# magic-research/vector_quantization

Hardware: AMD Instinct MI355X
Metric: quantized tokens/sec, VQGAN quantizer forward K=16384 D=256 (higher is better)
Workload: dtype f16+f32; 1 GPU; VQGAN K=16384 D=256, 256x256 images -> 16x16 tokens, bf16 latents, VQGANQuantizer.forward of the drop-in nn.Module, eval mode (prepare+argmin+gather+STE+loss); images_per_gpu=2048, parallelism=dp1 (independent shards, no data-path collective)

## Files before the change

### include/vqhip.h

```cpp
#ifndef VQHIP_H_
#define VQHIP_H_

#include <stddef.h>
#include <stdint.h>

#ifdef __cplusplus
extern "C" {
#endif

#define VQHIP_VERSION 600

#define VQHIP_METRIC_L2 0
#define VQHIP_METRIC_COS 1
#define VQHIP_METRIC_COS_BF16 5

#define VQHIP_DTYPE_F32 0
#define VQHIP_DTYPE_BF16 1

#define VQHIP_OK 0
#define VQHIP_EINVAL (-22)
#define VQHIP_ELAUNCH (-5)
#define VQHIP_ERCCL (-71)

int vqhip_version(void);
// ... 104 lines not shown
                          int64_t N, int64_t K, int D, int metric, int64_t *col_idx, void *ws, int64_t ws_bytes, void *stream);
int vqhip_cvq_pack(const int32_t *hist, int64_t numel, const void *x, int x_dtype, const int64_t *col_idx, const int32_t *count,
                   int64_t cap, int64_t K, int D, float *packed, void *stream);
int vqhip_cvq_apply(const float *w_in, float *w_out, const float *p_in, float *p_out, const int32_t *hist, int64_t numel,
                    const void *x, int x_dtype, const int64_t *col_idx, const float *packed, int world, const int32_t *slot,
                    int64_t cap, int64_t K, int D, float ema_decay, float eps, void *stream);
#define VQHIP_SYNC_MAX_ROWS (1 << 24)
int vqhip_cvq_col_keys(const void *x, int x_dtype, const float *e, const int32_t *rows, const int32_t *count, int64_t cap,
                       const int64_t *col_idx, int64_t N, int64_t K, int D, int metric, int rank, int64_t *keys, void *stream);
int vqhip_cvq_pack_sync(const int32_t *hist, int64_t numel, const void *x, int x_dtype, const int64_t *keys, const int32_t *count,
                        int64_t cap, int rank, int64_t K, int D, float *packed, void *stream);
int vqhip_allreduce_min_i64(int64_t *buf, int64_t n, void *comm, void *stream);
#define VQHIP_STEP_BEFORE_EXCHANGE 1
#define VQHIP_STEP_AFTER_EXCHANGE 2
#define VQHIP_STEP_ALL 3
#define VQHIP_STEP_PACK_SYNC 4
typedef struct vqhip_cvq_forward_t {
    int64_t struct_bytes;
    int64_t N, K;
    int32_t D, x_dtype, metric, world;
    float ema_decay, eps, beta;
    int32_t phases, exchange, list_ready, prefetch;
    int32_t anchor_sync, rank;
    int64_t cap;
    const void *x;
    const float *w_in, *p_in;
    float *w_out, *p_out;
    int32_t *rows, *slot, *count;
    int32_t *count_host;
    void *count_event;
    void *comm;
    void *cb; int64_t cb_bytes;
    int64_t *idx; int32_t *hist; float *xq;
    float *packed; int64_t packed_floats;
    float *z_ste, *mse; void *scratch16;
    void *ws; int64_t ws_bytes;
    int64_t cap_used, exchange_floats;
    unsigned long long *early_word_host;
    int32_t *early_seq_dev;
    int64_t *keys;
} vqhip_cvq_forward_t;
int64_t vqhip_cvq_forward_ws_bytes(int64_t N, int64_t K, int D, int64_t cap_max);
int vqhip_cvq_forward(vqhip_cvq_forward_t *args, void *stream);

typedef struct vqhip_vqkd_forward_t {
    int64_t struct_bytes;
    int64_t N, K;
    int32_t D, x_dtype, metric, world;
    float ema_decay;
    int32_t phases, exchange, ordered, tail, reserved0;
    const void *x;
    const float *w_in;
    float *w_mid, *w_out;
    float *xn, *xq;
    void *comm;
    void *cb; int64_t cb_bytes;
    int64_t *idx; int32_t *hist;
    float *packed; int64_t packed_floats;
    float *z_ste, *mse; void *scratch16;
    void *ws; int64_t ws_bytes;
    int64_t exchange_floats;
} vqhip_vqkd_forward_t;
int64_t vqhip_vqkd_forward_ws_bytes(int64_t N, int64_t K, int D);
int vqhip_vqkd_forward(vqhip_vqkd_forward_t *args, void *stream);
int vqhip_vqkd_backward(const void *x, int x_dtype, const float *xn, const float *w, const int64_t *idx, int64_t N, int D,
                        const float *g_zste, const float *g_loss, float *grad_x, void *stream);

typedef struct vqhip_vq_forward_t {
    int64_t struct_bytes;
    int64_t N, K;
    int32_t D, x_dtype, metric, normalize;
    float beta;
    int32_t reserved0;
    const void *x;
    const float *w_in;
    float *w_out, *xn;
    void *cb; int64_t cb_bytes;
    int64_t *idx; int32_t *hist; float *xq;
    float *z_ste, *mse; void *scratch16;
    void *ws; int64_t ws_bytes;
} vqhip_vq_forward_t;
int vqhip_vq_forward(vqhip_vq_forward_t *args, void *stream);

int vqhip_gather_rows(const void *x, int x_dtype, const int64_t *row_idx, int64_t K, int D, float *out,
                      void *stream);

int vqhip_diff(const void *a, int a_dtype, const void *b, int b_dtype, int64_t n, float scale,
               const float *scale_dev , float *out, double *sse,
               void *stream);
int vqhip_vq_backward(const void *x, int x_dtype, const float *e, const int64_t *idx, int64_t N, int D,
                      const float *g_zste, const float *g_cb, const float *g_cm, float *grad_x, float *grad_w,
                      void *stream);
int vqhip_vq_backward_ex(const void *x, int x_dtype, const float *e, const int64_t *idx, int64_t N, int D,
                         const float *g_zste, const float *g_cb, const float *g_cm, const float *g_comb, float beta,
                         float *grad_x, float *grad_w, void *stream);
int vqhip_vq_backward_map(const void *x_rows, int x_dtype, const float *e, const int64_t *idx, int64_t B, int64_t HW, int D,
                          const float *g_map, const float *g_cm, const float *g_comb, float beta, void *grad_map, int grad_dtype,
                          void *stream);
int vqhip_ste(const void *x, int x_dtype, const float *z, int64_t n, float *out, void *stream);
int vqhip_normalize_rows_bwd(const void *v, int dtype, const float *g, int64_t R, int D, float eps, float *gv,
                             void *stream);

int64_t vqhip_order_workspace_bytes(int64_t N, int64_t K);
int64_t vqhip_segsum_workspace_bytes(int64_t N, int D);
int vqhip_token_order(const int64_t *idx, int64_t N, int64_t K, int32_t *counts, int32_t *offsets, int32_t *order, void *ws,
                      int64_t ws_bytes, void *stream);
int vqhip_segsum_rows(const float *src, const int64_t *idx, const int32_t *order, const int32_t *offsets, int64_t N, int64_t K,
                      int D, float *dst, void *ws, int64_t ws_bytes, void *stream);
int vqhip_vq_backward_w_ordered(const void *x, int x_dtype, const float *e, const int64_t *idx, const int32_t *order,
                                const int32_t *offsets, int64_t N, int64_t K, int D, const float *g_cb, float *grad_w, void *ws,
                                int64_t ws_bytes, void *stream);

int vqhip_transpose(const void *in, void *out, int elem_bytes, int64_t B, int R, int C, void *stream);
int vqhip_codebook_metrics(const int64_t *counts, int64_t K, double *out, void *stream);

int vqhip_argmin_stats(const void *ws, int32_t *out, void *stream);

int vqhip_debug_proposal_scores(const void *x, int x_dtype, const void *cb, int64_t N, int64_t K, int D, int metric,
                                float *scores, float *margin, float *scale, void *ws, int64_t ws_bytes, void *stream);

int vqhip_profile_enable(int on);
int vqhip_set_tuning(int key, int value);
int vqhip_profile_collect(double *ms_sum, int64_t *launches);

#ifdef __cplusplus
}
#endif
#endif
```

### vector_quantization_amd/_lib.py

```python
from __future__ import annotations

import ctypes
import os
import subprocess

_HERE = os.path.dirname(os.path.abspath(__file__))
LIB_PATH = os.environ.get('VQHIP_LIB') or os.path.join(_HERE, 'libvqhip.so')

ABI_VERSION = 600
METRIC_L2, METRIC_COS, METRIC_COS_BF16 = 0, 1, 5
DTYPE_F32, DTYPE_BF16 = 0, 1
DTYPE_I32, DTYPE_I64 = 2, 3
LAYOUT_ROWS, LAYOUT_MAP = 0, 1
FSQ_MAX_C = 16

_vp, _i64, _i32, _f32 = ctypes.c_void_p, ctypes.c_int64, ctypes.c_int, ctypes.c_float


class CvqForwardArgs(ctypes.Structure):
    _fields_ = [('struct_bytes', _i64), ('N', _i64), ('K', _i64),
                ('D', _i32), ('x_dtype', _i32), ('metric', _i32), ('world', _i32),
                ('ema_decay', _f32), ('eps', _f32), ('beta', _f32),
                ('phases', _i32), ('exchange', _i32), ('list_ready', _i32), ('prefetch', _i32), ('anchor_sync', _i32), ('rank', _i32),
                ('cap', _i64),
                ('x', _vp), ('w_in', _vp), ('p_in', _vp), ('w_out', _vp), ('p_out', _vp),
                ('rows', _vp), ('slot', _vp), ('count', _vp), ('count_host', _vp), ('count_event', _vp), ('comm', _vp),
                ('cb', _vp), ('cb_bytes', _i64), ('idx', _vp), ('hist', _vp), ('xq', _vp),
                ('packed', _vp), ('packed_floats', _i64),
                ('z_ste', _vp), ('mse', _vp), ('scratch16', _vp),
                ('ws', _vp), ('ws_bytes', _i64),
                ('cap_used', _i64), ('exchange_floats', _i64),
                ('early_word_host', _vp), ('early_seq_dev', _vp), ('keys', _vp)]


class VqkdForwardArgs(ctypes.Structure):
    _fields_ = [('struct_bytes', _i64), ('N', _i64), ('K', _i64),
                ('D', _i32), ('x_dtype', _i32), ('metric', _i32), ('world', _i32),
                ('ema_decay', _f32),
                ('phases', _i32), ('exchange', _i32), ('ordered', _i32), ('tail', _i32), ('reserved0', _i32),
                ('x', _vp), ('w_in', _vp), ('w_mid', _vp), ('w_out', _vp), ('xn', _vp), ('xq', _vp), ('comm', _vp),
                ('cb', _vp), ('cb_bytes', _i64), ('idx', _vp), ('hist', _vp),
                ('packed', _vp), ('packed_floats', _i64),
                ('z_ste', _vp), ('mse', _vp), ('scratch16', _vp),
                ('ws', _vp), ('ws_bytes', _i64),
                ('exchange_floats', _i64)]


class VqForwardArgs(ctypes.Structure):
    _fields_ = [('struct_bytes', _i64), ('N', _i64), ('K', _i64),
                ('D', _i32), ('x_dtype', _i32), ('metric', _i32), ('normalize', _i32),
                ('beta', _f32), ('reserved0', _i32),
                ('x', _vp), ('w_in', _vp), ('w_out', _vp), ('xn', _vp),
                ('cb', _vp), ('cb_bytes', _i64), ('idx', _vp), ('hist', _vp), ('xq', _vp),
                ('z_ste', _vp), ('mse', _vp), ('scratch16', _vp),
                ('ws', _vp), ('ws_bytes', _i64)]


class FsqConstants(ctypes.Structure):
    _fields_ = [('struct_bytes', _i64), ('C', _i32), ('levels', _i32 * FSQ_MAX_C),
                ('shift', _f32 * FSQ_MAX_C), ('scale', _f32 * FSQ_MAX_C)]


STEP_BEFORE_EXCHANGE, STEP_AFTER_EXCHANGE, STEP_ALL, STEP_PACK_SYNC = 1, 2, 3, 4

SIGNATURES = {
    'vqhip_version': (_i32, []),
    'vqhip_last_error': (ctypes.c_char_p, []),
    'vqhip_codebook_bytes': (_i64, [_i64, _i32]),
    'vqhip_codebook_exact_offset': (_i64, [_i64, _i32]),
    'vqhip_encode': (_i32, [_vp, _i32, _vp, _i64, _i64, _i32, _i32, _vp, _i64, _vp, _vp, _vp, _vp, _i64, _vp]),
    'vqhip_encode_ex': (_i32, [_vp, _i32, _vp, _i64, _i64, _i32, _i32, _vp, _i64, _vp, _vp, _vp, _vp, _i64, _i32, _vp]),
    'vqhip_encode_map': (_i32, [_vp, _i32, _vp, _i64, _i64, _i64, _i32, _i32, _vp, _i64, _vp, _vp, _vp, _vp, _vp, _i64, _i32, _vp]),
    'vqhip_gather_ste_map': (_i32, [_vp, _i32, _vp, _vp, _i64, _i64, _i32, _vp, _vp, _f32, _vp, _vp]),
    'vqhip_workspace_bytes': (_i64, [_i64, _i64, _i32]),
    'vqhip_col_workspace_bytes': (_i64, [_i64, _i64, _i32]),
    'vqhip_codebook_prepare': (_i32, [_vp, _i64, _i32, _i32, _vp, _i64, _vp]),
    'vqhip_argmin': (_i32, [_vp, _i32, _vp, _vp, _i64, _i64, _i64, _i32, _i32, _vp, _vp, _vp, _i64, _vp]),
    'vqhip_argmin_exact': (_i32, [_vp, _i32, _vp, _i64, _i64, _i32, _i32, _vp, _vp, _vp, _vp, _i64, _vp]),
    'vqhip_distance': (_i32, [_vp, _i32, _vp, _i64, _i64, _i32, _i32, _vp, _vp, _i64, _vp]),
    'vqhip_col_argmin': (_i32, [_vp, _i32, _vp, _i64, _i64, _i32, _i32, _vp, _vp, _i64, _vp]),
    'vqhip_row_sqnorm': (_i32, [_vp, _i32, _i64, _i32, _vp, _vp]),
    'vqhip_normalize_rows': (_i32, [_vp, _i32, _i64, _i32, _f32, _vp, _vp]),
    'vqhip_gather_ste_loss': (_i32, [_vp, _i32, _vp, _vp, _i64, _i32, _vp, _vp, _vp, _vp]),
    'vqhip_gather_ste_mse': (_i32, [_vp, _i32, _vp, _vp, _i64, _i32, _vp, _vp, _vp, _f32, _vp, _vp]),
    'vqhip_hist': (_i32, [_vp, _i64, _i64, _vp, _vp]),
    'vqhip_hist_i32': (_i32, [_vp, _i64, _i64, _vp, _vp]),
    'vqhip_fsq_encode': (_i32, [ctypes.POINTER(FsqConstants), _vp, _i32, _i32, _i64, _i64, _vp, _vp, _i32, _vp, _vp, _vp]),
    'vqhip_fsq_backward': (_i32, [ctypes.POINTER(FsqConstants), _vp, _i32, _i32, _i64, _i64, _vp, _vp, _vp]),
    'vqhip_fsq_decode': (_i32, [ctypes.POINTER(FsqConstants), _vp, _i32, _i32, _i64, _i64, _vp, _vp]),
    'vqhip_entropy_workspace_bytes': (_i64, [_i64, _i64]),
    'vqhip_entropy_rows': (_i32, [_vp, _i64, _i64, _f32, _vp, _vp, _vp, _i32, _vp, _i64, _vp]),
    'vqhip_entropy_finish': (_i32, [_vp, _vp, _vp, _i64, _i64, _vp, _vp, _vp, _vp]),
    'vqhip_entropy_grad': (_i32, [_vp, _i64, _i64, _f32, _vp, _vp, _vp, _f32, _vp, _i32, _vp, _vp, _i32, _vp, _i64, _vp]),
    'vqhip_scatter_add_rows': (_i32, [_vp, _vp, _i64, _i64, _i32, _vp, _vp]),
    'vqhip_vqkd_update': (_i32, [_vp, _vp, _vp, _i64, _i32, _f32, _i32, _vp]),
    'vqhip_cvq_update': (_i32, [_vp, _vp, _vp, _i64, _vp, _vp, _i64, _i32, _f32, _f32, _i32, _vp]),
    'vqhip_gather_rows': (_i32, [_vp, _i32, _vp, _i64, _i32, _vp, _vp]),
    'vqhip_diff': (_i32, [_vp, _i32, _vp, _i32, _i64, _f32, _vp, _vp, _vp, _vp]),
    'vqhip_vq_backward': (_i32, [_vp, _i32, _vp, _vp, _i64, _i32, _vp, _vp, _vp, _vp, _vp, _vp]),
    'vqhip_vq_backward_ex': (_i32, [_vp, _i32, _vp, _vp, _i64, _i32, _vp, _vp, _vp, _vp, _f32, _vp, _vp, _vp]),
    'vqhip_vq_backward_map': (_i32, [_vp, _i32, _vp, _vp, _i64, _i64, _i32, _vp, _vp, _vp, _f32, _vp, _i32, _vp]),
    'vqhip_ste': (_i32, [_vp, _i32, _vp, _i64, _vp, _vp]),
    'vqhip_normalize_rows_bwd': (_i32, [_vp, _i32, _vp, _i64, _i32, _f32, _vp, _vp]),
    'vqhip_transpose': (_i32, [_vp, _vp, _i32, _i64, _i32, _i32, _vp]),
    'vqhip_codebook_metrics': (_i32, [_vp, _i64, _vp, _vp]),
    'vqhip_argmin_stats': (_i32, [_vp, _vp, _vp]),
    'vqhip_cvq_step': (_i32, [_vp, _vp, _vp, _vp, _vp, _i64, _vp, _i32, _vp, _i64, _i32, _f32, _f32, _vp]),
    'vqhip_cvq_decay': (_i32, [_vp, _i64, _f32, _f32, _vp, _vp]),
    'vqhip_cvq_update_rows': (_i32, [_vp, _vp, _vp, _vp, _i64, _i64, _i32, _f32, _f32, _vp]),
    'vqhip_pack_floats': (_i64, [_i64, _i64, _i32]),
    'vqhip_pack_counts': (_i32, [_vp, _i32, _i64, _i64, _vp, _vp]),
    'vqhip_unpack_counts': (_i32, [_vp, _i64, _vp, _vp]),
    'vqhip_cvq_rows': (_i32, [_vp, _i64, _f32, _f32, _vp, _vp, _vp, _vp]),
    'vqhip_col_rows_workspace_bytes': (_i64, [_i64, _i64, _i32]),
    'vqhip_col_argmin_rows': (_i32, [_vp, _i32, _vp, _vp, _vp, _i64, _i64, _i64, _i32, _i32, _vp, _vp, _i64, _vp]),
    'vqhip_cvq_pack': (_i32, [_vp, _i64, _vp, _i32, _vp, _vp, _i64, _i64, _i32, _vp, _vp]),
    'vqhip_cvq_forward_ws_bytes': (_i64, [_i64, _i64, _i32, _i64]),
    'vqhip_cvq_forward': (_i32, [ctypes.POINTER(CvqForwardArgs), _vp]),
    'vqhip_vqkd_forward_ws_bytes': (_i64, [_i64, _i64, _i32]),
    'vqhip_vqkd_forward': (_i32, [ctypes.POINTER(VqkdForwardArgs), _vp]),
    'vqhip_vq_forward': (_i32, [ctypes.POINTER(VqForwardArgs), _vp]),
    'vqhip_vqkd_backward': (_i32, [_vp, _i32, _vp, _vp, _vp, _i64, _i32, _vp, _vp, _vp, _vp]),
    'vqhip_cvq_apply': (_i32, [_vp, _vp, _vp, _vp, _vp, _i64, _vp, _i32, _vp, _vp, _i32, _vp, _i64, _i64, _i32, _f32, _f32, _vp]),
    'vqhip_cvq_col_keys': (_i32, [_vp, _i32, _vp, _vp, _vp, _i64, _vp, _i64, _i64, _i32, _i32, _i32, _vp, _vp]),
    'vqhip_cvq_pack_sync': (_i32, [_vp, _i64, _vp, _i32, _vp, _vp, _i64, _i32, _i64, _i32, _vp, _vp]),
    'vqhip_allreduce_min_i64': (_i32, [_vp, _i64, _vp, _vp]),
    'vqhip_order_workspace_bytes': (_i64, [_i64, _i64]),
    'vqhip_token_order': (_i32, [_vp, _i64, _i64, _vp, _vp, _vp, _vp, _i64, _vp]),
    'vqhip_segsum_workspace_bytes': (_i64, [_i64, _i32]),
    'vqhip_segsum_rows': (_i32, [_vp, _vp, _vp, _vp, _i64, _i64, _i32, _vp, _vp, _i64, _vp]),
    'vqhip_vq_backward_w_ordered': (_i32, [_vp, _i32, _vp, _vp, _vp, _vp, _i64, _i64, _i32, _vp, _vp, _vp, _i64, _vp]),
    'vqhip_debug_proposal_scores': (_i32, [_vp, _i32, _vp, _i64, _i64, _i32, _i32, _vp, _vp, _vp, _vp, _i64, _vp]),
    'vqhip_rccl_load': (_i32, [ctypes.c_char_p]),
    'vqhip_rccl_unique_id': (_i32, [_vp]),
    'vqhip_rccl_comm_init': (_i32, [ctypes.POINTER(_vp), _i32, _vp, _i32]),
    'vqhip_rccl_comm_destroy': (_i32, [_vp]),
    'vqhip_allreduce_packed': (_i32, [_vp, _i64, _vp, _vp]),
    'vqhip_profile_enable': (_i32, [_i32]),
    'vqhip_set_tuning': (_i32, [_i32, _i32]),
    'vqhip_profile_collect': (_i32, [ctypes.POINTER(ctypes.c_double), ctypes.POINTER(ctypes.c_int64)]),
}

_lib = None


class VqhipError(RuntimeError):
    pass


def build(verbose: bool = False) -> str:
    script = os.path.join(_HERE, 'csrc', 'build.sh')
    res = subprocess.run(['bash', script], capture_output=True, text=True)
    if res.returncode != 0:
        raise VqhipError(f'hipcc build of libvqhip.so failed:\n{res.stdout}\n{res.stderr}')
    if verbose:
        print(res.stdout.strip())
    return LIB_PATH


def lib() -> ctypes.CDLL:
    global _lib
    if _lib is None:
        if not os.path.exists(LIB_PATH):
            raise VqhipError(
                f'{LIB_PATH} not found: build it with vector_quantization_amd/csrc/build.sh '
                '(or __graft_entry__.build()); there is no fallback path')
        L = ctypes.CDLL(LIB_PATH)
# ... 20 lines not shown
```

### vector_quantization_amd/csrc/vqhip.hip

```cpp
#include "vqhip.h"

#include <hip/hip_runtime.h>
#include <stdio.h>
#include <string.h>

#include "vqhip_kernels.h"
#include "vqhip_fsq_kernels.h"
#include "vqhip_entropy_kernels.h"

static thread_local char g_err[256] = "";

static int fail(int code, const char *what, const char *detail = "") {
    snprintf(g_err, sizeof(g_err), "%s%s%s", what, detail[0] ? ": " : "", detail);
    return code;
}

#define VQ_CHECK_LAUNCH(name)                                            \
    do {                                                                 \
        hipError_t err__ = hipGetLastError();                            \
        if (err__ != hipSuccess) return fail(VQHIP_ELAUNCH, name, hipGetErrorString(err__)); \
    } while (0)

#define VQ_HIP(call)                                                     \
    do {                                                                 \
        hipError_t err__ = (call);                                       \
        if (err__ != hipSuccess) return fail(VQHIP_ELAUNCH, #call, hipGetErrorString(err__)); \
    } while (0)

#include <atomic>
#include <mutex>
#include <vector>
static std::atomic<bool> g_prof_on{false};
static std::mutex g_prof_mu;
static std::vector<std::pair<hipEvent_t, hipEvent_t>> g_prof_events;
static size_t g_prof_used = 0;

static long prof_begin(hipStream_t s) {
    if (!g_prof_on.load(std::memory_order_relaxed)) return -1;
    std::lock_guard<std::mutex> lock(g_prof_mu);
    if (g_prof_used == g_prof_events.size()) {
        hipEvent_t a, b;
        if (hipEventCreate(&a) != hipSuccess || hipEventCreate(&b) != hipSuccess) { g_prof_on = false; return -1; }
        g_prof_events.emplace_back(a, b);
    }
    const long slot = (long)g_prof_used++;
    (void)hipEventRecord(g_prof_events[slot].first, s);
    return slot;
}
static void prof_end(long slot, hipStream_t s) {
    if (slot < 0) return;
    std::lock_guard<std::mutex> lock(g_prof_mu);
    if ((size_t)slot < g_prof_events.size()) (void)hipEventRecord(g_prof_events[slot].second, s);
}

#define VQ_MAX_DEVICES 64
typedef std::atomic<size_t> LdsCache[VQ_MAX_DEVICES];
static int ensure_dyn_lds(const void *kern, size_t bytes, LdsCache &set) {
    int dev = 0;
    VQ_HIP(hipGetDevice(&dev));
    const bool cached = dev >= 0 && dev < VQ_MAX_DEVICES;
    if (!cached || bytes > set[dev].load(std::memory_order_acquire)) {
        VQ_HIP(hipFuncSetAttribute(kern, hipFuncAttributeMaxDynamicSharedMemorySize, (int)bytes));
        if (cached) {
            size_t cur = set[dev].load(std::memory_order_relaxed);
            while (cur < bytes && !set[dev].compare_exchange_weak(cur, bytes, std::memory_order_release)) {}
        }
    }
    return VQHIP_OK;
}

#define VQ_NEED(what, have, need)                                                                         \
    do {                                                                                                  \
        const int64_t need__ = (need);                                                                    \
        if ((have) < need__) {                                                                            \
            char msg__[160];                                                                              \
            snprintf(msg__, sizeof(msg__), "%lld bytes given, %lld needed", (long long)(have), (long long)need__); \
            return fail(VQHIP_EINVAL, what, msg__);                                                       \
        }                                                                                                 \
    } while (0)

static inline int waves_grid(int64_t rows, int waves_per_block) {
    return (int)((rows + waves_per_block - 1) / waves_per_block);
}

static std::atomic<int> g_tune_slices{0};
static std::atomic<int> g_tune_force_exact{0};
static std::atomic<int> g_tune_stream{1};
#define VQ_FUSED_DECIDE_MAX_N 16384

template <int NSTEP, int TT, int WAVES, int TPS, int NBUF = 2, bool FILTER = false, bool NOAUX = false, bool GROUPS = false, int XD = 0>
static int launch_coarse_cfg(const char *ximg, int64_t N, const char *frag, int64_t nstages, int nslices, float *rec,
                             int64_t Np, const VqCbStats *cbst, const float *xh2, const float *rho2, int Dp, int metric,
                             const VqDecideOut &dec, int pad_stage, int tpb, hipStream_t s) {
    constexpr int LDS = NBUF * (TPS * NSTEP + VQ_AUX_CHUNKS(TPS)) * VQ_CHUNK_BYTES;
    auto kern = coarse_kernel<NSTEP, TT, WAVES, TPS, NBUF, FILTER, NOAUX, GROUPS, XD>;
    static LdsCache lds_set;
    if (int rc = ensure_dyn_lds((const void *)kern, LDS, lds_set)) return rc;
    const int64_t ntiles = (N + 15) / 16;
    const int64_t ntb = (ntiles + tpb - 1) / tpb;
    const int grid = (int)(ntb * nslices);
    const long slot = prof_begin(s);
    kern<<<grid, WAVES * 64, LDS, s>>>(ximg, N, frag, nstages, nslices, rec, Np, cbst, xh2, rho2, Dp, metric, dec, pad_stage, tpb);
    prof_end(slot, s);
    VQ_CHECK_LAUNCH("coarse_kernel");
    return VQHIP_OK;
}

template <int TT, int WAVES, int TPS, int NBUF, bool NOAUX, int KS>
static int launch_coarse32_cfg(const char *ximg, int64_t N, const char *frag, int64_t nstages, int nslices, float *rec,
                               int64_t Np, const VqCbStats *cbst, const float *xh2, const float *rho2, int Dp, int metric,
                               const int *n_dev, const VqGroupLists &grp, int pad_stage, int tpb, hipStream_t s) {
    constexpr int LDS = NBUF * (TPS * 2 + VQ_AUX_CHUNKS(TPS)) * VQ_CHUNK_BYTES;
    auto kern = coarse32_kernel<TT, WAVES, TPS, NBUF, NOAUX, KS, VQ_GROUP_TILES>;
    static LdsCache lds_set;
    if (int rc = ensure_dyn_lds((const void *)kern, LDS, lds_set)) return rc;
    const int64_t ntiles = (N + 15) / 16;
    const int64_t ntb = (ntiles + tpb - 1) / tpb;
    const long slot = prof_begin(s);
    kern<<<(int)(ntb * nslices), WAVES * 64, LDS, s>>>(ximg, N, frag, nstages, nslices, rec, Np, cbst, xh2, rho2, Dp, metric, n_dev, grp, pad_stage, tpb);
    prof_end(slot, s);
    VQ_CHECK_LAUNCH("coarse32_kernel");
    return VQHIP_OK;
}

template <int NSTEP, int TT, int WAVES, int TPS, int NBUF = 2, int XD = 0>
static int launch_rescan_cfg(const char *ximg, const char *frag, int64_t nstages, const int *rescan_list, const int *counters,
                             const float *thr, int *rescan_cnt, int *cand_list, hipStream_t s, const void *xrows = nullptr) {
    constexpr int LDS = NBUF * (TPS * NSTEP + VQ_AUX_CHUNKS(TPS)) * VQ_CHUNK_BYTES + WAVES * TT * 16 * 4 * (1 + VQ_RESCAN_LOCAL);
    auto kern = rescan_kernel<NSTEP, TT, WAVES, TPS, NBUF, XD>;
    static LdsCache lds_set;
    if (int rc = ensure_dyn_lds((const void *)kern, LDS, lds_set)) return rc;
    kern<<<256, WAVES * 64, LDS, s>>>(ximg, frag, nstages, rescan_list, counters, thr, rescan_cnt, cand_list, xrows);
    VQ_CHECK_LAUNCH("rescan_kernel");
    return VQHIP_OK;
}

#ifndef VQ_W32_MAX_D
#define VQ_W32_MAX_D 32
#endif
#ifndef VQ_NBUF_D32
#define VQ_NBUF_D32 4
#endif
#ifndef VQ_D32_SMALL_TT
#define VQ_D32_SMALL_TT 2
#define VQ_D32_SMALL_W 8
#endif
#ifndef VQ_MIN_SLICES_FILTER
#define VQ_MIN_SLICES_FILTER 1
#endif
static int balanced_tiles_per_block(int64_t N, int full) {
    if (full < 16) return full;
    const int64_t ntiles = (N + 15) / 16;
    int best = full;
    int64_t best_cost = ((ntiles + full - 1) / full + 255) / 256 * full;
    for (int tpb = full - 1; tpb >= full / 2 && tpb >= 8; --tpb) {
        const int64_t cost = ((ntiles + tpb - 1) / tpb + 255) / 256 * tpb;
        if (cost < best_cost) { best_cost = cost; best = tpb; }
    }
    return best;
}

static bool vq_xdirect(int64_t N, int64_t K, int D, int x_dtype, int metric, const int *n_dev) {
    if (D != 256 || n_dev != nullptr || vq_cb_layout(K, D).nstages < 2 || g_tune_slices.load() == 1) return false;
    if (x_dtype != VQHIP_DTYPE_BF16) return false;
    if (metric != VQHIP_METRIC_L2 && metric != VQHIP_METRIC_COS && metric != VQHIP_METRIC_COS_BF16) return false;
    if (N <= VQ_FUSED_DECIDE_MAX_N) return false;
    return !(N <= 4096 || (N <= 256 * 64 && K <= 4096));
}

static int pick_slices(int64_t ntb, int64_t nstages, int min_slices = 2) {
    if (const int forced = g_tune_slices.load(); forced > 0) { int ns = forced; while (ns > 1 && ns > nstages) ns >>= 1; return ns; }
    int64_t want = (256 + ntb - 1) / ntb;
    want = want < min_slices ? min_slices : want;
    int ns = 1;
    while (ns < want && ns < VQ_MAX_SLICES) ns <<= 1;
    while (ns > 1 && ns > nstages) ns >>= 1;
    return ns;
}

struct VqGroupRun { int used, ks, noaux, pad_stage; };
static int launch_coarse(const char *ximg, int64_t N, const VqCbLayout &L, const char *frag, float *rec, int64_t Np,
                         const VqCbStats *cbst, const float *xh2, const float *rho2, int metric, const VqDecideOut &dec,
                         int *nslices_out, int *fused_decide_out, hipStream_t s, VqGroupLists grp = VqGroupLists{nullptr, nullptr, nullptr, nullptr, 0, 1, 0},
                         VqGroupRun *grun = nullptr, bool xd = false) {
    const int nstep = L.nstep;
    const bool small = N <= 256 * 64;
    const bool small16 = N <= 4096 || (N <= 256 * 64 && L.K <= 4096);
    const bool small32 = N < 512 * 512;
    const bool noaux = !VQ_IS_L2(metric);
    const int pad_stage = (L.K % ((int64_t)L.tps * VQ_TILE_CODES)) ? (int)(L.nstages - 1) : -1;
#define VQ_CFG(NS, TT, W, ...)                                                                      \
    {                                                                                               \
        int64_t ntb = (N + (W) * (TT) * 16 - 1) / ((W) * (TT) * 16);                                \
        int ns = pick_slices(ntb, L.nstages, (NS) <= 8 ? VQ_MIN_SLICES_FILTER : 2);                 \
        *nslices_out = ns;                                                                          \
        const int tpb = (ns == 1) ? balanced_tiles_per_block(N, (W) * (TT)) : (W) * (TT);           \
        VqDecideOut dsel = dec;                                                                     \
        if (!(ns == 1 || N <= VQ_FUSED_DECIDE_MAX_N)) dsel.idx = nullptr;                           \
        *fused_decide_out = dsel.idx != nullptr ? 1 : 0;                                            \
        return launch_coarse_cfg<NS, TT, W, __VA_ARGS__>(ximg, N, frag, L.nstages, ns, rec, Np, cbst, xh2, rho2, L.Dp, metric, dsel, pad_stage, tpb, s); \
    }
    switch (nstep) {
        case 2: if ((L.D <= 16 || (L.D <= VQ_W32_MAX_D && noaux)) && N >= VQ_W32_MIN_N && grp.bcnt != nullptr && grun != nullptr) {
                    const int tt = small32 ? 1 : 2;
                    const int full = 8 * tt * 2;
                    const int64_t ntb0 = (N + full * 16 - 1) / (full * 16);
                    int ns = pick_slices(ntb0, L.nstages, VQ_MIN_SLICES_FILTER);
                    ns = ns > VQ_GROUP_MAX_SLICES ? VQ_GROUP_MAX_SLICES : ns;
                    *nslices_out = ns;
                    int tpb = (ns == 1) ? balanced_tiles_per_block(N, full) : full;
                    tpb = (tpb + 1) & ~1;
                    *fused_decide_out = 0;
                    grun->used = 1; grun->ks = L.D <= 16 ? 1 : 2; grun->noaux = noaux ? 1 : 0; grun->pad_stage = pad_stage;
#define VQ_CFG32(TTW, NOAUXV, KSV) return launch_coarse32_cfg<TTW, 8, VQ_TPS_D32, VQ_NBUF_D32, NOAUXV, KSV>(ximg, N, frag, L.nstages, ns, rec, Np, cbst, xh2, rho2, L.Dp, metric, dec.n_dev, grp, pad_stage, tpb, s)
                    if (L.D <= 16) {
                        if (tt == 1) { if (noaux) VQ_CFG32(1, true, 1); else VQ_CFG32(1, false, 1); }
                        else { if (noaux) VQ_CFG32(2, true, 1); else VQ_CFG32(2, false, 1); }
                    } else {
                        if (tt == 1) { if (noaux) VQ_CFG32(1, true, 2); else VQ_CFG32(1, false, 2); }
                        else { if (noaux) VQ_CFG32(2, true, 2); else VQ_CFG32(2, false, 2); }
                    }
#undef VQ_CFG32
                }
                if (N >= VQ_GROUPS_MIN_N) {
                    if (noaux) { if (small32) VQ_CFG(2, VQ_D32_SMALL_TT, VQ_D32_SMALL_W, VQ_TPS_D32, VQ_NBUF_D32, true, true, true) else VQ_CFG(2, 4, 8, VQ_TPS_D32, VQ_NBUF_D32, true, true, true) }
                    if (small32) VQ_CFG(2, VQ_D32_SMALL_TT, VQ_D32_SMALL_W, VQ_TPS_D32, VQ_NBUF_D32, true, false, true) else VQ_CFG(2, 4, 8, VQ_TPS_D32, VQ_NBUF_D32, true, false, true)
                }
                if (noaux) { if (small32) VQ_CFG(2, VQ_D32_SMALL_TT, VQ_D32_SMALL_W, VQ_TPS_D32, VQ_NBUF_D32, true, true) else VQ_CFG(2, 4, 8, VQ_TPS_D32, VQ_NBUF_D32, true, true) }
                if (small32) VQ_CFG(2, VQ_D32_SMALL_TT, VQ_D32_SMALL_W, VQ_TPS_D32, VQ_NBUF_D32, true) else VQ_CFG(2, 4, 8, VQ_TPS_D32, VQ_NBUF_D32, true)
        case 4: if (small) VQ_CFG(4, 2, 8, 4, 4, true) else VQ_CFG(4, 4, 8, 4, 4, true)
        case 8: if (small) VQ_CFG(8, 2, 8, 4, 4, true) else VQ_CFG(8, 4, 8, 4, 4, true)
        case 16: if (xd && !small16) VQ_CFG(16, 4, 8, VQ_TPS16, 4, false, false, false, 1)
                 if (small16) VQ_CFG(16, 2, 8, VQ_TPS16, 4) else VQ_CFG(16, 4, 8, VQ_TPS16, 4)
        case 32: VQ_CFG(32, 2, 8, 2)
        case 48: VQ_CFG(48, 2, 8, 1)
        case 64: {
            auto cost = [&](int tokens, double eff) {
                const int64_t ntb = (N + tokens - 1) / tokens;
                const int ns = pick_slices(ntb, L.nstages, 2);
                return (double)((ntb * ns + 255) / 256) * tokens * ((double)L.nstages / ns) / eff;
            };
            if (cost(192, 1.18) < cost(128, 1.0)) VQ_CFG(64, 3, 4, 1) else VQ_CFG(64, 1, 8, 1)
        }
        default: break;
    }
#undef VQ_CFG
    return fail(VQHIP_EINVAL, "vqhip_argmin: unsupported padded D");
}

static int resident_grid(int per_cu) {
    static std::atomic<int> cus[VQ_MAX_DEVICES];
    int dev = 0, n = 0;
    if (hipGetDevice(&dev) != hipSuccess) return 256 * per_cu;
    if (dev >= 0 && dev < VQ_MAX_DEVICES && (n = cus[dev].load(std::memory_order_relaxed)) > 0) return n * per_cu;
    if (hipDeviceGetAttribute(&n, hipDeviceAttributeMultiprocessorCount, dev) != hipSuccess || n <= 0) n = 256;
    if (dev >= 0 && dev < VQ_MAX_DEVICES) cus[dev].store(n, std::memory_order_relaxed);
    return n * per_cu;
}

template <int MODE>
static int run_exact_tiled(const void *x, int x_dtype, const float *e, const float *en, const float *xn, int64_t N, int64_t K,
                           int D, int metric, u64 *keys, float *dout, hipStream_t s) {
    const int bf = x_dtype == VQHIP_DTYPE_F32 ? 0 : 1;
    const int64_t items = ((N + 127) / 128) * ((K + 255) / 256);
    if (g_tune_stream.load() && D % (bf ? 8 : 4) == 0 && items < (int64_t)1 << 31) {
        static LdsCache ssets[2];
        const int lds = vq_xs_lds_bytes(bf);
        const void *kern = bf ? (const void *)exact_stream_kernel<1, MODE> : (const void *)exact_stream_kernel<0, MODE>;
        if (int rc = ensure_dyn_lds(kern, lds, ssets[bf])) return rc;
        const int cap = resident_grid(2);
        const int grid = (int)(items < cap ? items : cap);
        if (bf) exact_stream_kernel<1, MODE><<<grid, 256, lds, s>>>(x, e, en, xn, N, K, D, metric, keys, dout);
        else exact_stream_kernel<0, MODE><<<grid, 256, lds, s>>>(x, e, en, xn, N, K, D, metric, keys, dout);
        VQ_CHECK_LAUNCH("exact_stream_kernel");
        return VQHIP_OK;
    }
    constexpr int LDS = 2 * 32 * 128 * 4 + 8 * 32 * 4;
    static LdsCache sets[4];
    const void *kerns[4] = {(const void *)exact_tiled_kernel<0, MODE, false>, (const void *)exact_tiled_kernel<1, MODE, false>,
                            (const void *)exact_tiled_kernel<0, MODE, true>, (const void *)exact_tiled_kernel<1, MODE, true>};
    const int v4 = (D % 4 == 0) ? 2 : 0;
// ... 78 lines not shown
}

static int launch_vqkd_front(const float *w_in, float *w_mid, int64_t K, const void *x, int x_dtype, float *xn, int64_t N, int D, float eps,
                             float *zero, int64_t nzero, int w_passes, hipStream_t s) {
    if (D <= 32) {
        const int L = D <= 8 ? 8 : (D <= 16 ? 16 : 32), rpb = 4 * (64 / L);
        const int kblocks = (int)((K + rpb - 1) / rpb), xblocks = (int)((N + rpb - 1) / rpb);
#define VQ_FRONT_SMALL(DT, LL) vqkd_front_small_kernel<DT, LL><<<kblocks + xblocks, 256, 0, s>>>(w_in, w_mid, K, x, xn, N, D, eps, kblocks, zero, nzero, w_passes)
        if (x_dtype == VQHIP_DTYPE_F32) { if (L == 8) VQ_FRONT_SMALL(0, 8); else if (L == 16) VQ_FRONT_SMALL(0, 16); else VQ_FRONT_SMALL(0, 32); }
        else { if (L == 8) VQ_FRONT_SMALL(1, 8); else if (L == 16) VQ_FRONT_SMALL(1, 16); else VQ_FRONT_SMALL(1, 32); }
#undef VQ_FRONT_SMALL
    } else {
        const int kblocks = (int)((K + 3) / 4), xblocks = (int)((N + 3) / 4);
        if (x_dtype == VQHIP_DTYPE_F32) vqkd_front_kernel<0><<<kblocks + xblocks, 256, 0, s>>>(w_in, w_mid, K, x, xn, N, D, eps, kblocks, zero, nzero, w_passes);
        else vqkd_front_kernel<1><<<kblocks + xblocks, 256, 0, s>>>(w_in, w_mid, K, x, xn, N, D, eps, kblocks, zero, nzero, w_passes);
    }
    VQ_CHECK_LAUNCH("vqkd_front_kernel");
    return VQHIP_OK;
}

int64_t vqhip_codebook_bytes(int64_t K, int D) {
    if (K <= 0 || D <= 0) return 0;
    return vq_cb_layout(K, D).total;
}

int64_t vqhip_workspace_bytes(int64_t N, int64_t K, int D) {
    if (N < 0 || K <= 0 || D <= 0) return 0;
    return vq_ws_layout(N > 0 ? N : 1, K, D).total;
}

int vqhip_row_sqnorm(const void *v, int dtype, int64_t R, int D, float *out, void *stream) {
    if (!v || !out || D <= 0 || R < 0) return fail(VQHIP_EINVAL, "vqhip_row_sqnorm: bad argument");
    if (R == 0) return VQHIP_OK;
    hipStream_t s = (hipStream_t)stream;
    if (D <= 32 && (dtype == VQHIP_DTYPE_F32 || dtype == VQHIP_DTYPE_BF16)) return launch_row_small<false>(v, dtype, R, D, 0.0f, out, s);
    if (dtype == VQHIP_DTYPE_F32) row_sqnorm_kernel<0><<<waves_grid(R, 4), 256, 0, s>>>(v, R, D, out);
    else if (dtype == VQHIP_DTYPE_BF16) row_sqnorm_kernel<1><<<waves_grid(R, 4), 256, 0, s>>>(v, R, D, out);
    else return fail(VQHIP_EINVAL, "vqhip_row_sqnorm: dtype");
    VQ_CHECK_LAUNCH("row_sqnorm_kernel");
    return VQHIP_OK;
}

int vqhip_normalize_rows(const void *v, int dtype, int64_t R, int D, float eps, float *out, void *stream) {
    if (!v || !out || D <= 0 || R < 0) return fail(VQHIP_EINVAL, "vqhip_normalize_rows: bad argument");
    if (R == 0) return VQHIP_OK;
    hipStream_t s = (hipStream_t)stream;
    if (D <= 32 && (dtype == VQHIP_DTYPE_F32 || dtype == VQHIP_DTYPE_BF16)) return launch_row_small<true>(v, dtype, R, D, eps, out, s);
    if (dtype == VQHIP_DTYPE_F32) normalize_rows_kernel<0><<<waves_grid(R, 4), 256, 0, s>>>(v, R, D, eps, out);
    else if (dtype == VQHIP_DTYPE_BF16) normalize_rows_kernel<1><<<waves_grid(R, 4), 256, 0, s>>>(v, R, D, eps, out);
    else return fail(VQHIP_EINVAL, "vqhip_normalize_rows: dtype");
    VQ_CHECK_LAUNCH("normalize_rows_kernel");
    return VQHIP_OK;
}

static int codebook_prepare_impl(const float *e, int64_t K, int D, int metric, void *cb, void *stream) {
    if (K >= (1ll << 31)) return fail(VQHIP_EINVAL, "vqhip_codebook_prepare: K too large");
    hipStream_t s = (hipStream_t)stream;
    VqCbLayout L = vq_cb_layout(K, D);
    char *c = (char *)cb;
    if (VQ_IS_COS(metric) && vq_coarse_supported(D)) {
        cb_cos_kernel<<<(int)(L.nstages * L.tps), 256, 0, s>>>(e, K, D, metric, c, L);
        VQ_CHECK_LAUNCH("cb_cos_kernel");
        return VQHIP_OK;
    }
    cb_stats_kernel<<<(int)((K + 15) / 16), 256, 0, s>>>(e, K, D, metric, c, L);
    VQ_CHECK_LAUNCH("cb_stats_kernel");
    if (vq_coarse_supported(D)) {
        cb_image_kernel<<<(int)(L.nstages * L.tps), 256, 0, s>>>(e, K, D, metric, c, L);
        VQ_CHECK_LAUNCH("cb_image_kernel");
    }
    return VQHIP_OK;
}

int vqhip_codebook_prepare(const float *e, int64_t K, int D, int metric, void *cb, int64_t cb_bytes, void *stream) {
    if (!e || !cb || K <= 0 || D <= 0 || (metric != VQHIP_METRIC_L2 && metric != VQHIP_METRIC_COS && metric != VQHIP_METRIC_COS_BF16))
        return fail(VQHIP_EINVAL, "vqhip_codebook_prepare: bad argument");
    VQ_NEED("vqhip_codebook_prepare: cb too small", cb_bytes, vqhip_codebook_bytes(K, D));
    return codebook_prepare_impl(e, K, D, metric, cb, stream);
}

int vqhip_argmin_exact(const void *x, int x_dtype, const float *e, int64_t N, int64_t K, int D, int metric, int64_t *idx,
                       float *dmin, int32_t *hist, void *ws, int64_t ws_bytes, void *stream);

static int argmin_pipeline(const void *x, int x_dtype, const float *e_exact, const void *cb, int64_t N, int64_t K, int D,
                           int metric, int64_t *idx, int32_t *hist, void *ws, void *stream, bool x_prepared = false,
                           const int *n_dev = nullptr) {
    hipStream_t s = (hipStream_t)stream;
    VqCbLayout L = vq_cb_layout(K, D);
    VqWsLayout W = vq_ws_layout(N, K, D);
    const char *c = (const char *)cb;
    char *w = (char *)ws;
    const int64_t Np = (N + 63) / 64 * 64;
    int *counters = (int *)(w + W.off_counters);
    float *xh2 = (float *)(w + W.off_xh2), *rho2 = (float *)(w + W.off_rho2), *rec = (float *)(w + W.off_rec);
    int *flag_list = (int *)(w + W.off_flag);
    u64 *keys = (u64 *)(w + W.off_keys);
    const float *en = (const float *)(c + L.off_en);

    int nslices = 1, rc;
    char *ximg = w + W.off_ximg;
    int *rescan_list = flag_list;
    int *multi_list = (int *)(w + W.off_multi), *exact_list = (int *)(w + W.off_exact);
    float *thr = (float *)(w + W.off_thr);
    int *rescan_cnt = (int *)(w + W.off_rcnt), *cand_list = (int *)(w + W.off_rlist);
    int *arrive = (int *)(w + W.off_arrive);
    const int narrive = (int)W.narrive;
    int xgrid = (int)((N + 31) / 32);
    const bool xd = vq_xdirect(N, K, D, x_dtype, metric, n_dev);
    if (!x_prepared) {
        if (xd) xgrid = xgrid < 64 ? xgrid : 64;
        if (x_dtype == VQHIP_DTYPE_F32) x_prep_kernel<0><<<xgrid, 256, 0, s>>>(x, N, D, L.nstep, ximg, xh2, rho2, (float *)(w + W.off_xn), counters, (char *)cb, L, arrive, narrive, xd);
        else x_prep_kernel<1><<<xgrid, 256, 0, s>>>(x, N, D, L.nstep, ximg, xh2, rho2, (float *)(w + W.off_xn), counters, (char *)cb, L, arrive, narrive, xd);
        VQ_CHECK_LAUNCH("x_prep_kernel");
    }
    VqDecideOut dec{idx, hist, rescan_list, multi_list, exact_list, counters, keys, thr, rescan_cnt, arrive, n_dev,
                    x, xh2, rho2, (float *)(w + W.off_xn)};
    VqDecideOut dec_arg = dec;
    int fused_done = 0;
    VqGroupLists grp{nullptr, nullptr, nullptr, nullptr, 0, 1, 0};
    VqGroupRun grun{0, 0, 0, -1};
    const int ntiles_cb = (int)(L.nstages * L.tps);
    int nbuckets = 0;
    if (W.nbkt > 0 && ntiles_cb <= VQ_GROUP_MAX_TILES && N < (1ll << 30)) {
        grp.R = vq_group_replicas(ntiles_cb / VQ_GROUP_TILES);
        nbuckets = ntiles_cb / VQ_GROUP_TILES * grp.R;
        grp.bcnt = (int *)(w + W.off_bcnt);
        grp.blist = (uint32_t *)(w + W.off_blist);
        grp.bfrag = w + W.off_bfrag;
        grp.rece2 = (float *)(w + W.off_rece2);
        grp.cap = (int)(W.blist_entries / nbuckets / 32 * 32);
        uint32_t bits = 1;
        while ((1u << bits) < (uint32_t)(ntiles_cb / VQ_GROUP_TILES)) ++bits;
        grp.idmask = (1u << bits) - 1u;
    }
    rc = launch_coarse(ximg, N, L, c + L.off_frag, rec, Np, (const VqCbStats *)(c + L.off_stats), xh2, rho2, metric, dec_arg, &nslices, &fused_done, s, grp, &grun, xd);
    if (rc) return rc;
    const float *rece2 = nullptr;
    if (grun.used) {
        const int igrid = (nbuckets + 3) / 4;
        if (grun.ks == 1) identify32_kernel<1, VQ_GROUP_TILES><<<igrid, 256, 0, s>>>(c + L.off_frag, L.nstages, nslices, nbuckets, rec, Np, (const VqCbStats *)(c + L.off_stats), grp, grun.pad_stage, grun.noaux);
        else identify32_kernel<2, VQ_GROUP_TILES><<<igrid, 256, 0, s>>>(c + L.off_frag, L.nstages, nslices, nbuckets, rec, Np, (const VqCbStats *)(c + L.off_stats), grp, grun.pad_stage, grun.noaux);
        VQ_CHECK_LAUNCH("identify32_kernel");
        rece2 = grp.rece2;
    }
    if (!fused_done) {
        refine_decide_kernel<<<(int)((N + 1023) / 1024), 1024, 0, s>>>(c, L, N, metric, nslices, rec, xh2, rho2, Np, dec, rece2);
        VQ_CHECK_LAUNCH("refine_decide_kernel");
    }
    float *xnorm = (float *)(w + W.off_xn);
    {
        const char *frag = c + L.off_frag;
        int rrc = VQHIP_OK;
        if (xd) rrc = launch_rescan_cfg<16, 2, 8, VQ_TPS16, 4, 1>(ximg, frag, L.nstages, rescan_list, counters, thr, rescan_cnt, cand_list, s, x);
        else switch (L.nstep) {
#define VQ_RESCAN(NS, TT, ...) case NS: rrc = launch_rescan_cfg<NS, TT, 8, __VA_ARGS__>(ximg, frag, L.nstages, rescan_list, counters, thr, rescan_cnt, cand_list, s); break;
            VQ_RESCAN(2, 2, VQ_TPS_D32, 4) VQ_RESCAN(4, 2, 4, 4) VQ_RESCAN(8, 2, 4, 4) VQ_RESCAN(16, 2, VQ_TPS16, 4) VQ_RESCAN(32, 2, 2) VQ_RESCAN(48, 2, 1) VQ_RESCAN(64, 1, 1)
#undef VQ_RESCAN
            default: return fail(VQHIP_EINVAL, "vqhip_argmin: unsupported padded D");
        }
        if (rrc) return rrc;
        VQ_CHECK_LAUNCH("rescan_kernel");
    }
    {
        int S0 = 4;
        while (S0 < 2 * nslices) S0 <<= 1;
        const int64_t g0 = 2048, g1 = 1024;
        if (x_dtype == VQHIP_DTYPE_F32)
            refine_rerank_kernel<0><<<(int)(g0 + g1), 256, 0, s>>>(x, e_exact, c, L, D, metric, nslices, S0, (int)g0, rec, xh2, rho2,
                                                                  xnorm, Np, idx, hist, multi_list, rescan_list, counters,
                                                                  rescan_cnt, cand_list, exact_list, keys, grun.used);
        else
            refine_rerank_kernel<1><<<(int)(g0 + g1), 256, 0, s>>>(x, e_exact, c, L, D, metric, nslices, S0, (int)g0, rec, xh2, rho2,
                                                                  xnorm, Np, idx, hist, multi_list, rescan_list, counters,
                                                                  rescan_cnt, cand_list, exact_list, keys, grun.used);
        VQ_CHECK_LAUNCH("refine_rerank_kernel");
    }
    if (const int force = g_tune_force_exact.load()) {
        force_exact_rows_kernel<<<1, 1024, 0, s>>>((int)(force < N ? force : N), exact_list, counters, keys);
        VQ_CHECK_LAUNCH("force_exact_rows_kernel");
    }
    return run_exact_rows(x, x_dtype, e_exact, en, xnorm, N, K, D, metric, exact_list, counters + 2, keys, counters + 3, idx, hist, s);
}

static int encode_fused_front(const void *rows, int rows_dtype, int64_t N, const float *codes, int64_t Kc, int D, int cb_metric,
                              void *cb, void *ws, bool xnorm, float *xq, hipStream_t s, int32_t *hist_zero = nullptr,
                              int64_t hw = 0, void *xrows = nullptr, const int32_t *grows = nullptr, const int32_t *gcount = nullptr) {
    VqCbLayout L = vq_cb_layout(Kc, D);
    VqWsLayout W = vq_ws_layout(N, Kc, D);
    char *w = (char *)ws, *c = (char *)cb;
    const bool cosimg = VQ_IS_COS(cb_metric) || (cb_metric & 3) == VQ_METRIC_DOT;
    const int nblk_stats = cosimg ? (int)(L.nstages * L.tps) : (int)((Kc + 15) / 16);
    const int toff = (!xnorm && hw == 0 && grows == nullptr && vq_xdirect(N, Kc, D, rows_dtype, cb_metric, nullptr)) ? 1 : 0;
    int xgrid = (int)((N + 31) / 32);
    if (toff) xgrid = xgrid < 64 ? xgrid : 64;
    const int narrive = (int)W.narrive;
    int *counters = (int *)(w + W.off_counters), *arrive = (int *)(w + W.off_arrive);
    float *xh2 = (float *)(w + W.off_xh2), *rho2 = (float *)(w + W.off_rho2), *xn = (float *)(w + W.off_xn);
    char *ximg = w + W.off_ximg;
#define VQ_PRE(DT, XN, MAP, COSI) pre_kernel<DT, XN, MAP, COSI><<<nblk_stats + xgrid, 256, 0, s>>>(codes, Kc, cb_metric, c, L, nblk_stats, rows, N, D, L.nstep, ximg, xh2, rho2, xn, counters, arrive, narrive, xq, 1e-12f, hist_zero, hw, xrows, nullptr, nullptr, toff)
#define VQ_PRE2(DT, XN, MAP) do { if (cosimg) VQ_PRE(DT, XN, MAP, true); else VQ_PRE(DT, XN, MAP, false); } while (0)
    if (grows != nullptr) {
        if (rows_dtype != VQHIP_DTYPE_F32 || xnorm || hw > 0 || L.nstep == 2) return fail(VQHIP_EINVAL, "encode_fused_front: gather form");
        if (cosimg) pre_kernel<0, false, false, true, true><<<nblk_stats + xgrid, 256, 0, s>>>(codes, Kc, cb_metric, c, L, nblk_stats, rows, N, D, L.nstep, ximg, xh2, rho2, xn, counters, arrive, narrive, xq, 1e-12f, hist_zero, hw, xrows, grows, gcount);
        else pre_kernel<0, false, false, false, true><<<nblk_stats + xgrid, 256, 0, s>>>(codes, Kc, cb_metric, c, L, nblk_stats, rows, N, D, L.nstep, ximg, xh2, rho2, xn, counters, arrive, narrive, xq, 1e-12f, hist_zero, hw, xrows, grows, gcount);
    } else
    if (hw > 0) {
        if (rows_dtype == VQHIP_DTYPE_F32) { if (xnorm) VQ_PRE2(0, true, true); else VQ_PRE2(0, false, true); }
        else { if (xnorm) VQ_PRE2(1, true, true); else VQ_PRE2(1, false, true); }
    } else {
        if (rows_dtype == VQHIP_DTYPE_F32) { if (xnorm) VQ_PRE2(0, true, false); else VQ_PRE2(0, false, false); }
        else { if (xnorm) VQ_PRE2(1, true, false); else VQ_PRE2(1, false, false); }
    }
#undef VQ_PRE2
#undef VQ_PRE
    VQ_CHECK_LAUNCH("pre_kernel");
    if (cosimg) return VQHIP_OK;
    cb_image_kernel<<<(int)(L.nstages * L.tps), 256, 0, s>>>(codes, Kc, D, cb_metric, c, L);
    VQ_CHECK_LAUNCH("cb_image_kernel");
    return VQHIP_OK;
}

int vqhip_encode(const void *x, int x_dtype, const float *e, int64_t N, int64_t K, int D, int metric, void *cb, int64_t cb_bytes,
                 int64_t *idx, int32_t *hist, float *xq, void *ws, int64_t ws_bytes, void *stream) {
    return vqhip_encode_ex(x, x_dtype, e, N, K, D, metric, cb, cb_bytes, idx, hist, xq, ws, ws_bytes, 0, stream);
}

int vqhip_encode_ex(const void *x, int x_dtype, const float *e, int64_t N, int64_t K, int D, int metric, void *cb, int64_t cb_bytes,
                    int64_t *idx, int32_t *hist, float *xq, void *ws, int64_t ws_bytes, int flags, void *stream) {
    const bool zero_hist = hist != nullptr && (flags & VQHIP_ENCODE_ZERO_HIST) != 0;
    if (N == 0 || !vq_coarse_supported(D)) {
        if (zero_hist && K > 0) VQ_HIP(hipMemsetAsync(hist, 0, (size_t)K * 4, (hipStream_t)stream));
    }
    if (N == 0) return e && cb && K > 0 && D > 0 ? vqhip_codebook_prepare(e, K, D, metric, cb, cb_bytes, stream) : fail(VQHIP_EINVAL, "vqhip_encode: bad argument");
    if (!x || !e || !cb || !idx || !ws || N < 0 || K <= 0 || D <= 0) return fail(VQHIP_EINVAL, "vqhip_encode: bad argument");
    if (metric != VQHIP_METRIC_L2 && metric != VQHIP_METRIC_COS && metric != VQHIP_METRIC_COS_BF16) return fail(VQHIP_EINVAL, "vqhip_encode: metric");
    if (x_dtype != VQHIP_DTYPE_F32 && x_dtype != VQHIP_DTYPE_BF16) return fail(VQHIP_EINVAL, "vqhip_encode: x_dtype");
    if (VQ_IS_COS(metric) && !xq) return fail(VQHIP_EINVAL, "vqhip_encode: the cosine metric needs the xq buffer");
    if (N >= (1ll << 31) || K >= (1ll << 31)) return fail(VQHIP_EINVAL, "vqhip_encode: N or K too large");
    VQ_NEED("vqhip_encode: cb too small", cb_bytes, vqhip_codebook_bytes(K, D));
    VQ_NEED("vqhip_encode: ws too small", ws_bytes, vqhip_workspace_bytes(N, K, D));
    if (!vq_coarse_supported(D)) {
        if (int rc = vqhip_codebook_prepare(e, K, D, metric, cb, cb_bytes, stream)) return rc;
        const void *rows = x; int rows_dtype = x_dtype;
        if (VQ_IS_COS(metric)) {
            if (VQ_IS_BF16(metric)) return fail(VQHIP_EINVAL, "vqhip_encode: the bf16-autocast cosine metric needs D <= 1024, D % 8 == 0");
            if (int rc = vqhip_normalize_rows(x, x_dtype, N, D, 1e-12f, xq, stream)) return rc;
            rows = xq; rows_dtype = VQHIP_DTYPE_F32;
        }
        return vqhip_argmin(rows, rows_dtype, e, cb, cb_bytes, N, K, D, metric, idx, hist, ws, ws_bytes, stream);
    }
    hipStream_t s = (hipStream_t)stream;
    const bool cos = VQ_IS_COS(metric);
    if (int rc = encode_fused_front(x, x_dtype, N, e, K, D, metric, cb, ws, cos, xq, s, zero_hist ? hist : nullptr)) return rc;
    VqCbLayout L = vq_cb_layout(K, D);
    const float *e_exact = cos ? (const float *)((const char *)cb + L.off_eexact) : e;
    return argmin_pipeline(cos ? (const void *)xq : x, cos ? VQHIP_DTYPE_F32 : x_dtype, e_exact, cb, N, K, D, metric, idx, hist, ws,
                           stream, true);
}

int vqhip_encode_map(const void *x_map, int x_dtype, const float *e, int64_t B, int64_t HW, int64_t K, int D, int metric, void *cb,
                     int64_t cb_bytes, int64_t *idx, int32_t *hist, void *xrows, float *xq, void *ws, int64_t ws_bytes, int flags,
                     void *stream) {
    const int64_t N = B * HW;
    if (!x_map || !e || !cb || !idx || !xrows || !ws || B <= 0 || HW <= 0 || K <= 0 || D <= 0) return fail(VQHIP_EINVAL, "vqhip_encode_map: bad argument");
    if (VQ_IS_COS(metric) && !xq) return fail(VQHIP_EINVAL, "vqhip_encode_map: the cosine metric needs the xq buffer");
    if (metric != VQHIP_METRIC_L2 && metric != VQHIP_METRIC_COS && metric != VQHIP_METRIC_COS_BF16) return fail(VQHIP_EINVAL, "vqhip_encode_map: metric");
    if (x_dtype != VQHIP_DTYPE_F32 && x_dtype != VQHIP_DTYPE_BF16) return fail(VQHIP_EINVAL, "vqhip_encode_map: x_dtype");
    if (N >= (1ll << 31) || K >= (1ll << 31)) return fail(VQHIP_EINVAL, "vqhip_encode_map: N or K too large");
    if (!vq_coarse_supported(D)) return fail(VQHIP_EINVAL, "vqhip_encode_map: needs D <= 1024, D % 8 == 0 (transpose and use vqhip_encode)");
    VQ_NEED("vqhip_encode_map: cb too small", cb_bytes, vqhip_codebook_bytes(K, D));
    VQ_NEED("vqhip_encode_map: ws too small", ws_bytes, vqhip_workspace_bytes(N, K, D));
    hipStream_t s = (hipStream_t)stream;
    const bool cos = VQ_IS_COS(metric);
    const bool zero_hist = hist != nullptr && (flags & VQHIP_ENCODE_ZERO_HIST) != 0;
    if (int rc = encode_fused_front(x_map, x_dtype, N, e, K, D, metric, cb, ws, cos, cos ? xq : nullptr, s,
                                    zero_hist ? hist : nullptr, HW, xrows)) return rc;
    VqCbLayout L = vq_cb_layout(K, D);
    const float *e_exact = cos ? (const float *)((const char *)cb + L.off_eexact) : e;
    return argmin_pipeline(cos ? (const void *)xq : (const void *)xrows, cos ? VQHIP_DTYPE_F32 : x_dtype, e_exact, cb, N, K, D, metric,
                           idx, hist, ws, stream, true);
}

int vqhip_argmin(const void *x, int x_dtype, const float *e, const void *cb, int64_t cb_bytes, int64_t N, int64_t K, int D, int metric,
                 int64_t *idx, int32_t *hist, void *ws, int64_t ws_bytes, void *stream) {
    if (N == 0) return VQHIP_OK;
    if (!x || !cb || !idx || !ws || N < 0 || K <= 0 || D <= 0) return fail(VQHIP_EINVAL, "vqhip_argmin: bad argument");
    if (metric != VQHIP_METRIC_L2 && metric != VQHIP_METRIC_COS && metric != VQHIP_METRIC_COS_BF16) return fail(VQHIP_EINVAL, "vqhip_argmin: metric");
    if (x_dtype != VQHIP_DTYPE_F32 && x_dtype != VQHIP_DTYPE_BF16) return fail(VQHIP_EINVAL, "vqhip_argmin: x_dtype");
    if (metric == VQHIP_METRIC_L2 && !e) return fail(VQHIP_EINVAL, "vqhip_argmin: e is required for L2");
    if (N >= (1ll << 31) || K >= (1ll << 31)) return fail(VQHIP_EINVAL, "vqhip_argmin: N or K too large");
    VQ_NEED("vqhip_argmin: cb too small", cb_bytes, vqhip_codebook_bytes(K, D));
    VQ_NEED("vqhip_argmin: ws too small", ws_bytes, vqhip_workspace_bytes(N, K, D));
    VqCbLayout L = vq_cb_layout(K, D);
    const float *e_exact = VQ_IS_COS(metric) ? (const float *)((const char *)cb + L.off_eexact) : e;
    if (!vq_coarse_supported(D)) {
        VQ_HIP(hipMemsetAsync(ws, 0, 256, (hipStream_t)stream));
        return vqhip_argmin_exact(x, x_dtype, e_exact, N, K, D, metric, idx, nullptr, hist, ws, ws_bytes, stream);
    }
    return argmin_pipeline(x, x_dtype, e_exact, cb, N, K, D, metric, idx, hist, ws, stream);
}

int vqhip_argmin_exact(const void *x, int x_dtype, const float *e, int64_t N, int64_t K, int D, int metric, int64_t *idx,
                       float *dmin, int32_t *hist, void *ws, int64_t ws_bytes, void *stream) {
    if (N == 0) return VQHIP_OK;
    if (!x || !e || !idx || !ws || N < 0 || K <= 0 || D <= 0) return fail(VQHIP_EINVAL, "vqhip_argmin_exact: bad argument");
    if (x_dtype != VQHIP_DTYPE_F32 && x_dtype != VQHIP_DTYPE_BF16) return fail(VQHIP_EINVAL, "vqhip_argmin_exact: x_dtype");
    if (N >= (1ll << 31) || K >= (1ll << 31)) return fail(VQHIP_EINVAL, "vqhip_argmin_exact: N or K too large");
    VQ_NEED("vqhip_argmin_exact: ws too small", ws_bytes, vqhip_workspace_bytes(N, K, D));
    hipStream_t s = (hipStream_t)stream;
    VqWsLayout W = vq_ws_layout(N, K, D);
    char *w = (char *)ws;
    u64 *keys = (u64 *)(w + W.off_keys);
    float *en = (float *)(w + W.off_en);
    if (metric == VQHIP_METRIC_L2) {
        int rc = vqhip_row_sqnorm(e, VQHIP_DTYPE_F32, K, D, en, stream);
        if (rc) return rc;
    }
    fill_u64_kernel<<<256, 256, 0, s>>>(keys, N, ~0ull);
    VQ_CHECK_LAUNCH("fill_u64_kernel");
    float *xn = (float *)(w + W.off_xh2);
    if (metric == VQHIP_METRIC_L2) {
        int rc0 = vqhip_row_sqnorm(x, x_dtype, N, D, xn, stream);
        if (rc0) return rc0;
    }
    int rc = run_exact_tiled<0>(x, x_dtype, e, en, xn, N, K, D, metric, keys, nullptr, s);
    if (rc) return rc;
    finalize_kernel<<<256, 256, 0, s>>>(keys, nullptr, nullptr, N, idx, dmin, hist);
    VQ_CHECK_LAUNCH("finalize_kernel");
    return VQHIP_OK;
}

int64_t vqhip_col_workspace_bytes(int64_t N, int64_t K, int D) {
    if (N <= 0 || K <= 0 || D <= 0) return 0;
    int64_t a = (vq_ws_layout(K, N, D).total + 1023) / 1024 * 1024;
    int64_t b = (vq_cb_layout(N, D).total + 1023) / 1024 * 1024;
    int64_t legacy = vq_ws_layout(N, K, D).total;
    int64_t t = a + b + N * (int64_t)D * 4;
    return t > legacy ? t : legacy;
}

// ... 732 lines not shown
    VQ_NEED("vqhip_vqkd_forward: packed buffer too small (floats)", a->packed_floats, floats);
    int64_t o_counts, o_offsets, o_order, o_ows, o_sws, o_x2, total;
    vqkd_ws_offsets(N, K, D, &o_counts, &o_offsets, &o_order, &o_ows, &o_sws, &o_x2, &total);
    VQ_NEED("vqhip_vqkd_forward: ws too small", a->ws_bytes, total);
    hipStream_t s = (hipStream_t)stream;
    char *w = (char *)a->ws;
    float *payload = a->packed + VQ_PACK_HEADER(K);
    if (a->phases & VQHIP_STEP_BEFORE_EXCHANGE) {
        a->exchange_floats = floats;
        int64_t nzero = a->ordered ? 0 : K * (int64_t)D;
        if (nzero && ((K & 1) || (nzero % 4))) {
            VQ_HIP(hipMemsetAsync(payload, 0, (size_t)nzero * 4, s));
            nzero = 0;
        }
        if (int rc = launch_vqkd_front(a->w_in, a->w_mid, K, a->x, a->x_dtype, a->xn, N, D, 1e-12f, payload, nzero, 2, s)) return rc;
        const int xblocks = (int)((N + 3) / 4);
        if (int rc = vqhip_encode_ex(a->xn, VQHIP_DTYPE_F32, a->w_mid, N, K, D, a->metric, a->cb, a->cb_bytes, a->idx, a->hist, a->xq, a->ws,
                                     vq_align1k(vq_ws_layout(N, K, D).total), VQHIP_ENCODE_ZERO_HIST, stream)) return rc;
        const int hb = (int)((K + 255) / 256);
        if (a->ordered) {
            int32_t *counts = (int32_t *)(w + o_counts), *offsets = (int32_t *)(w + o_offsets), *order = (int32_t *)(w + o_order);
            if (int rc = vqhip_token_order(a->idx, N, K, counts, offsets, order, w + o_ows, vqhip_order_workspace_bytes(N, K), stream)) return rc;
            const float *x2 = a->xq;
            if (VQ_IS_BF16(a->metric)) {
                if (int rc = vqhip_normalize_rows(a->xn, VQHIP_DTYPE_F32, N, D, 1e-12f, (float *)(w + o_x2), stream)) return rc;
                x2 = (const float *)(w + o_x2);
            }
            if (int rc = vqhip_segsum_rows(x2, a->idx, order, offsets, N, K, D, payload, w + o_sws, vqhip_segsum_workspace_bytes(N, D), stream)) return rc;
            vqkd_scatter_pack_kernel<<<hb, 256, 0, s>>>(a->hist, N, a->xn, a->idx, N, K, D, 1e-12f, a->packed, hb, 0);
        } else {
            vqkd_scatter_pack_kernel<<<hb + xblocks, 256, 0, s>>>(a->hist, N, a->xn, a->idx, N, K, D, 1e-12f, a->packed, hb, 1);
        }
        VQ_CHECK_LAUNCH("vqkd_scatter_pack_kernel");
    }
    if (a->phases == VQHIP_STEP_ALL && a->exchange && a->comm)
        if (int rc = vqhip_allreduce_packed(a->packed, floats, a->comm, stream)) return rc;
    if (a->phases & VQHIP_STEP_AFTER_EXCHANGE) {
        vqkd_update_packed_kernel<<<waves_grid(K, 4), 256, 0, s>>>(a->w_mid, a->w_out, a->packed, K, D, a->ema_decay);
        VQ_CHECK_LAUNCH("vqkd_update_packed_kernel");
        if (a->tail) {
            double *tail_partials = (double *)((char *)a->ws + vq_ws_layout(N, K, D).off_rec);
            if (D <= 32) {
                const int L = D <= 8 ? 8 : (D <= 16 ? 16 : 32), rpb = 16 * (64 / L);
                int grid = (int)((N + rpb - 1) / rpb); grid = grid > 256 ? 256 : grid;
                if (L == 8) vqkd_tail_small_kernel<8><<<grid, 1024, 0, s>>>(a->xn, a->w_out, a->idx, N, D, 1e-12f, a->z_ste, (double *)a->scratch16, a->mse, tail_partials);
                else if (L == 16) vqkd_tail_small_kernel<16><<<grid, 1024, 0, s>>>(a->xn, a->w_out, a->idx, N, D, 1e-12f, a->z_ste, (double *)a->scratch16, a->mse, tail_partials);
                else vqkd_tail_small_kernel<32><<<grid, 1024, 0, s>>>(a->xn, a->w_out, a->idx, N, D, 1e-12f, a->z_ste, (double *)a->scratch16, a->mse, tail_partials);
            } else {
                int grid = (int)((N + 15) / 16); grid = grid > 256 ? 256 : grid;
                vqkd_tail_kernel<<<grid, 1024, 0, s>>>(a->xn, a->w_out, a->idx, N, D, 1e-12f, a->z_ste, (double *)a->scratch16, a->mse, tail_partials);
            }
            VQ_CHECK_LAUNCH("vqkd_tail_kernel");
        }
    }
    return VQHIP_OK;
}

int vqhip_vq_forward(vqhip_vq_forward_t *a, void *stream) {
    if (!a || a->struct_bytes != (int64_t)sizeof(vqhip_vq_forward_t)) return fail(VQHIP_EINVAL, "vqhip_vq_forward: struct_bytes != sizeof(vqhip_vq_forward_t)");
    const int64_t N = a->N, K = a->K;
    const int D = a->D;
    if (N <= 0 || K <= 0 || D <= 0 || N >= (1ll << 31) || K >= (1ll << 31)) return fail(VQHIP_EINVAL, "vqhip_vq_forward: N, K, D");
    if (a->metric != VQHIP_METRIC_L2 && a->metric != VQHIP_METRIC_COS && a->metric != VQHIP_METRIC_COS_BF16) return fail(VQHIP_EINVAL, "vqhip_vq_forward: metric");
    if (a->x_dtype != VQHIP_DTYPE_F32 && a->x_dtype != VQHIP_DTYPE_BF16) return fail(VQHIP_EINVAL, "vqhip_vq_forward: x_dtype");
    if (!a->x || !a->w_in || !a->cb || !a->idx || !a->ws || (a->normalize && (!a->w_out || !a->xn))) return fail(VQHIP_EINVAL, "vqhip_vq_forward: null pointer");
    if (VQ_IS_COS(a->metric) && !a->xq) return fail(VQHIP_EINVAL, "vqhip_vq_forward: the cosine metric needs the xq buffer");
    if ((a->z_ste || a->mse) && (!a->mse || !a->scratch16)) return fail(VQHIP_EINVAL, "vqhip_vq_forward: the decode tail needs mse and scratch16");
    VQ_NEED("vqhip_vq_forward: ws too small", a->ws_bytes, vqhip_workspace_bytes(N, K, D));
    hipStream_t s = (hipStream_t)stream;
    const void *rows = a->x;
    int rows_dtype = a->x_dtype;
    const float *codes = a->w_in;
    if (a->normalize) {
        if (int rc = launch_vqkd_front(a->w_in, a->w_out, K, a->x, a->x_dtype, a->xn, N, D, 1e-12f, nullptr, 0, 1, s)) return rc;
        rows = a->xn; rows_dtype = VQHIP_DTYPE_F32; codes = a->w_out;
    }
    if (int rc = vqhip_encode_ex(rows, rows_dtype, codes, N, K, D, a->metric, a->cb, a->cb_bytes, a->idx, a->hist, a->xq, a->ws, a->ws_bytes,
                                 a->hist ? VQHIP_ENCODE_ZERO_HIST : 0, stream)) return rc;
    if (a->mse)
        if (int rc = vqhip_gather_ste_mse(rows, rows_dtype, codes, a->idx, N, D, nullptr, a->z_ste, a->mse, a->beta, a->scratch16, stream)) return rc;
    return VQHIP_OK;
}

int vqhip_vqkd_backward(const void *x, int x_dtype, const float *xn, const float *w, const int64_t *idx, int64_t N, int D,
                        const float *g_zste, const float *g_loss, float *grad_x, void *stream) {
    if (!x || !xn || !w || !idx || !grad_x || N < 0 || D <= 0) return fail(VQHIP_EINVAL, "vqhip_vqkd_backward: bad argument");
    if (N == 0) return VQHIP_OK;
    hipStream_t s = (hipStream_t)stream;
    if (x_dtype != VQHIP_DTYPE_F32 && x_dtype != VQHIP_DTYPE_BF16) return fail(VQHIP_EINVAL, "vqhip_vqkd_backward: x_dtype");
    if (D <= 32) {
        const int L = D <= 8 ? 8 : (D <= 16 ? 16 : 32), rpb = 4 * (64 / L);
        int grid = (int)((N + rpb - 1) / rpb); grid = grid > 2048 ? 2048 : grid;
#define VQ_BWD_SMALL(DT, LL) vqkd_backward_small_kernel<DT, LL><<<grid, 256, 0, s>>>(x, xn, w, idx, N, D, 1e-12f, g_zste, g_loss, grad_x)
        if (x_dtype == VQHIP_DTYPE_F32) { if (L == 8) VQ_BWD_SMALL(0, 8); else if (L == 16) VQ_BWD_SMALL(0, 16); else VQ_BWD_SMALL(0, 32); }
        else { if (L == 8) VQ_BWD_SMALL(1, 8); else if (L == 16) VQ_BWD_SMALL(1, 16); else VQ_BWD_SMALL(1, 32); }
#undef VQ_BWD_SMALL
        VQ_CHECK_LAUNCH("vqkd_backward_kernel");
        return VQHIP_OK;
    }
    int grid = (int)((N + 3) / 4); grid = grid > 2048 ? 2048 : grid;
    if (x_dtype == VQHIP_DTYPE_F32) vqkd_backward_kernel<0><<<grid, 256, 0, s>>>(x, xn, w, idx, N, D, 1e-12f, g_zste, g_loss, grad_x);
    else vqkd_backward_kernel<1><<<grid, 256, 0, s>>>(x, xn, w, idx, N, D, 1e-12f, g_zste, g_loss, grad_x);
    VQ_CHECK_LAUNCH("vqkd_backward_kernel");
    return VQHIP_OK;
}

int vqhip_argmin_stats(const void *ws, int32_t *out, void *stream) {
    if (!ws || !out) return fail(VQHIP_EINVAL, "vqhip_argmin_stats: bad argument");
    VQ_HIP(hipMemcpyAsync(out, ws, 16, hipMemcpyDeviceToDevice, (hipStream_t)stream));
    return VQHIP_OK;
}

int vqhip_diff(const void *a, int a_dtype, const void *b, int b_dtype, int64_t n, float scale, const float *scale_dev,
               float *out, double *sse, void *stream) {
    if (!a || !b || n < 0 || (!out && !sse)) return fail(VQHIP_EINVAL, "vqhip_diff: bad argument");
    if (n == 0) return VQHIP_OK;
    hipStream_t s = (hipStream_t)stream;
    int grid = (int)((n + 255) / 256); grid = grid > 2048 ? 2048 : grid;
    if (a_dtype == 0 && b_dtype == 0) diff_kernel<0, 0><<<grid, 256, 0, s>>>(a, b, n, scale, scale_dev, out, sse);
    else if (a_dtype == 0 && b_dtype == 1) diff_kernel<0, 1><<<grid, 256, 0, s>>>(a, b, n, scale, scale_dev, out, sse);
    else if (a_dtype == 1 && b_dtype == 0) diff_kernel<1, 0><<<grid, 256, 0, s>>>(a, b, n, scale, scale_dev, out, sse);
    else if (a_dtype == 1 && b_dtype == 1) diff_kernel<1, 1><<<grid, 256, 0, s>>>(a, b, n, scale, scale_dev, out, sse);
    else return fail(VQHIP_EINVAL, "vqhip_diff: dtype");
    VQ_CHECK_LAUNCH("diff_kernel");
    return VQHIP_OK;
}

int vqhip_vq_backward(const void *x, int x_dtype, const float *e, const int64_t *idx, int64_t N, int D, const float *g_zste,
                      const float *g_cb, const float *g_cm, float *grad_x, float *grad_w, void *stream) {
    return vqhip_vq_backward_ex(x, x_dtype, e, idx, N, D, g_zste, g_cb, g_cm, nullptr, 0.0f, grad_x, grad_w, stream);
}

int vqhip_vq_backward_ex(const void *x, int x_dtype, const float *e, const int64_t *idx, int64_t N, int D, const float *g_zste,
                         const float *g_cb, const float *g_cm, const float *g_comb, float beta, float *grad_x, float *grad_w,
                         void *stream) {
    if (!x || !e || !idx || N < 0 || D <= 0 || (!grad_x && !grad_w)) return fail(VQHIP_EINVAL, "vqhip_vq_backward: bad argument");
    if (N == 0) return VQHIP_OK;
    hipStream_t s = (hipStream_t)stream;
    int grid = (int)((N + 3) / 4); grid = grid > 2048 ? 2048 : grid;
    if (x_dtype == VQHIP_DTYPE_F32)
        vq_backward_kernel<0><<<grid, 256, 0, s>>>(x, e, idx, N, D, g_zste, g_cb, g_cm, grad_x, grad_w, g_comb, beta);
    else if (x_dtype == VQHIP_DTYPE_BF16)
        vq_backward_kernel<1><<<grid, 256, 0, s>>>(x, e, idx, N, D, g_zste, g_cb, g_cm, grad_x, grad_w, g_comb, beta);
    else return fail(VQHIP_EINVAL, "vqhip_vq_backward: x_dtype");
    VQ_CHECK_LAUNCH("vq_backward_kernel");
    return VQHIP_OK;
}

int vqhip_vq_backward_map(const void *x_rows, int x_dtype, const float *e, const int64_t *idx, int64_t B, int64_t HW, int D,
                          const float *g_map, const float *g_cm, const float *g_comb, float beta, void *grad_map, int grad_dtype,
                          void *stream) {
    if (!x_rows || !e || !idx || !grad_map || B <= 0 || HW <= 0 || D <= 0) return fail(VQHIP_EINVAL, "vqhip_vq_backward_map: bad argument");
    if ((HW % 256) != 0 || (D % 32) != 0) return fail(VQHIP_EINVAL, "vqhip_vq_backward_map: needs HW % 256 == 0 and D % 32 == 0 (transpose and use vqhip_vq_backward_ex)");
    if ((x_dtype != VQHIP_DTYPE_F32 && x_dtype != VQHIP_DTYPE_BF16) || (grad_dtype != VQHIP_DTYPE_F32 && grad_dtype != VQHIP_DTYPE_BF16))
        return fail(VQHIP_EINVAL, "vqhip_vq_backward_map: dtype");
    const int64_t N = B * HW, nt = N / 256;
    int csplit = 1;
    while (nt * csplit < 512 && (D / 32) % (csplit * 2) == 0) csplit *= 2;
    const int64_t items = nt * csplit;
    const int grid = (int)(items < 1024 ? items : 1024);
    constexpr int LDS = 2 * 32 * 256 * 4;
    static LdsCache sets[4];
    const int v = (x_dtype == VQHIP_DTYPE_BF16 ? 1 : 0) + (grad_dtype == VQHIP_DTYPE_BF16 ? 2 : 0);
    const void *kerns[4] = {(const void *)vq_backward_map256_kernel<0, 0>, (const void *)vq_backward_map256_kernel<1, 0>,
                            (const void *)vq_backward_map256_kernel<0, 1>, (const void *)vq_backward_map256_kernel<1, 1>};
    if (int rc = ensure_dyn_lds(kerns[v], LDS, sets[v])) return rc;
// ... 59 lines not shown
        return fail(VQHIP_EINVAL, "vqhip_vq_backward_w_ordered: bad argument (D must be a multiple of 4)");
    VQ_NEED("vqhip_vq_backward_w_ordered: ws too small", ws_bytes, vqhip_segsum_workspace_bytes(N, D));
    if (x_dtype != VQHIP_DTYPE_F32 && x_dtype != VQHIP_DTYPE_BF16) return fail(VQHIP_EINVAL, "vqhip_vq_backward_w_ordered: x_dtype");
    return run_segsum<1>(x, x_dtype, e, idx, order, offsets, N, K, D, g_cb, grad_w, ws, (hipStream_t)stream);
}

int vqhip_ste(const void *x, int x_dtype, const float *z, int64_t n, float *out, void *stream) {
    if (!x || !z || !out || n < 0) return fail(VQHIP_EINVAL, "vqhip_ste: bad argument");
    if (n == 0) return VQHIP_OK;
    hipStream_t s = (hipStream_t)stream;
    int grid = (int)((n + 255) / 256); grid = grid > 4096 ? 4096 : grid;
    if (x_dtype == VQHIP_DTYPE_F32) ste_kernel<0><<<grid, 256, 0, s>>>(x, z, n, out);
    else if (x_dtype == VQHIP_DTYPE_BF16) ste_kernel<1><<<grid, 256, 0, s>>>(x, z, n, out);
    else return fail(VQHIP_EINVAL, "vqhip_ste: dtype");
    VQ_CHECK_LAUNCH("ste_kernel");
    return VQHIP_OK;
}

int vqhip_normalize_rows_bwd(const void *v, int dtype, const float *g, int64_t R, int D, float eps, float *gv, void *stream) {
    if (!v || !g || !gv || R < 0 || D <= 0) return fail(VQHIP_EINVAL, "vqhip_normalize_rows_bwd: bad argument");
    if (R == 0) return VQHIP_OK;
    hipStream_t s = (hipStream_t)stream;
    if (dtype == VQHIP_DTYPE_F32) normalize_bwd_kernel<0><<<waves_grid(R, 4), 256, 0, s>>>(v, g, R, D, eps, gv);
    else if (dtype == VQHIP_DTYPE_BF16) normalize_bwd_kernel<1><<<waves_grid(R, 4), 256, 0, s>>>(v, g, R, D, eps, gv);
    else return fail(VQHIP_EINVAL, "vqhip_normalize_rows_bwd: dtype");
    VQ_CHECK_LAUNCH("normalize_bwd_kernel");
    return VQHIP_OK;
}

int vqhip_transpose(const void *in, void *out, int elem_bytes, int64_t B, int R, int C, void *stream) {
    if (!in || !out || B < 0 || R <= 0 || C <= 0 || (elem_bytes != 2 && elem_bytes != 4))
        return fail(VQHIP_EINVAL, "vqhip_transpose: bad argument");
    if (B == 0) return VQHIP_OK;
    if (B > 65535) return fail(VQHIP_EINVAL, "vqhip_transpose: batch too large for one launch");
    dim3 grid((C + 63) / 64, (R + 63) / 64, (unsigned)B);
    hipStream_t s = (hipStream_t)stream;
    if (elem_bytes == 4) transpose_kernel<uint32_t><<<grid, 256, 0, s>>>((const uint32_t *)in, (uint32_t *)out, B, R, C);
    else transpose_kernel<uint16_t><<<grid, 256, 0, s>>>((const uint16_t *)in, (uint16_t *)out, B, R, C);
    VQ_CHECK_LAUNCH("transpose_kernel");
    return VQHIP_OK;
}

int vqhip_codebook_metrics(const int64_t *counts, int64_t K, double *out, void *stream) {
    if (!counts || !out || K <= 0) return fail(VQHIP_EINVAL, "vqhip_codebook_metrics: bad argument");
    codebook_metrics_kernel<<<1, 1024, 0, (hipStream_t)stream>>>(counts, K, out);
    VQ_CHECK_LAUNCH("codebook_metrics_kernel");
    return VQHIP_OK;
}

int vqhip_debug_proposal_scores(const void *x, int x_dtype, const void *cb, int64_t N, int64_t K, int D, int metric,
                                float *scores, float *margin, float *scale, void *ws, int64_t ws_bytes, void *stream) {
    if (!x || !cb || !scores || !margin || !scale || !ws || N <= 0 || K <= 0 || !vq_coarse_supported(D))
        return fail(VQHIP_EINVAL, "vqhip_debug_proposal_scores: bad argument");
    VQ_NEED("vqhip_debug_proposal_scores: ws too small", ws_bytes, vqhip_workspace_bytes(N, K, D));
    hipStream_t s = (hipStream_t)stream;
    VqCbLayout L = vq_cb_layout(K, D);
    VqWsLayout W = vq_ws_layout(N, K, D);
    const char *c = (const char *)cb;
    char *w = (char *)ws;
    int *counters = (int *)(w + W.off_counters);
    float *xh2 = (float *)(w + W.off_xh2), *rho2 = (float *)(w + W.off_rho2);
    char *ximg = w + W.off_ximg;
    const int xgrid = (int)((N + 31) / 32);
    if (x_dtype == VQHIP_DTYPE_F32) x_prep_kernel<0><<<xgrid, 256, 0, s>>>(x, N, D, L.nstep, ximg, xh2, rho2, (float *)(w + W.off_xn), counters, (char *)cb, L);
    else if (x_dtype == VQHIP_DTYPE_BF16) x_prep_kernel<1><<<xgrid, 256, 0, s>>>(x, N, D, L.nstep, ximg, xh2, rho2, (float *)(w + W.off_xn), counters, (char *)cb, L);
    else return fail(VQHIP_EINVAL, "vqhip_debug_proposal_scores: x_dtype");
    VQ_CHECK_LAUNCH("x_prep_kernel");
    const char *frag = c + L.off_frag;
    switch (L.nstep) {
#define VQ_DBG(NS, TPS) case NS: debug_scores_kernel<NS, TPS><<<512, 256, 0, s>>>(ximg, frag, L.nstages, N, K, scores); break;
        VQ_DBG(2, VQ_TPS_D32) VQ_DBG(4, 4) VQ_DBG(8, 4) VQ_DBG(16, VQ_TPS16) VQ_DBG(32, 2) VQ_DBG(48, 1) VQ_DBG(64, 1)
#undef VQ_DBG
        default: return fail(VQHIP_EINVAL, "vqhip_debug_proposal_scores: unsupported padded D");
    }
    VQ_CHECK_LAUNCH("debug_scores_kernel");
    debug_margin_kernel<<<(int)((N + 255) / 256), 256, 0, s>>>(c, L, N, metric, xh2, rho2, margin, scale);
    VQ_CHECK_LAUNCH("debug_margin_kernel");
    return VQHIP_OK;
}

int vqhip_set_tuning(int key, int value) {
    if (key == 2) g_tune_slices = (value == 1 || value == 2 || value == 4 || value == 8 || value == 16) ? value : 0;
    else if (key == 18) g_tune_stream = value != 0;
    else if (key == 12) g_tune_force_exact = value > 0 ? (value < 1024 ? value : 1024) : 0;
    else return fail(VQHIP_EINVAL, "vqhip_set_tuning: unknown key");
    return VQHIP_OK;
}

#include <dlfcn.h>
struct VqRcclId { char bytes[VQHIP_RCCL_ID_BYTES]; };
namespace {
struct RcclApi {
    void *handle = nullptr;
    int (*get_unique_id)(void *) = nullptr;
    int (*comm_init_rank)(void **, int, VqRcclId, int) = nullptr;
    int (*comm_destroy)(void *) = nullptr;
    int (*all_reduce)(const void *, void *, size_t, int, int, void *, hipStream_t) = nullptr;
    const char *(*error_string)(int) = nullptr;
};
}
static RcclApi g_rccl;
static std::mutex g_rccl_mu;
static const int kNcclFloat32 = 7, kNcclInt64 = 4, kNcclSum = 0, kNcclMin = 3;

static int rccl_fail(const char *what, int rc) {
    return fail(VQHIP_ERCCL, what, g_rccl.error_string ? g_rccl.error_string(rc) : "RCCL error");
}

int vqhip_rccl_load(const char *path) {
    std::lock_guard<std::mutex> lock(g_rccl_mu);
    if (g_rccl.handle) return VQHIP_OK;
    void *h = nullptr;
    if (path && path[0]) {
        h = dlopen(path, RTLD_NOW | RTLD_GLOBAL);
        if (!h) return fail(VQHIP_ERCCL, "vqhip_rccl_load: librccl.so not loadable", dlerror());
    } else {
        const char *names[] = {"librccl.so", "librccl.so.1"};
        for (const char *n : names)
            if (!h) h = dlopen(n, RTLD_NOW | RTLD_NOLOAD);
        if (!h) return fail(VQHIP_ERCCL, "vqhip_rccl_load: no librccl.so is mapped into this process under that name; pass the path of the copy the application uses");
    }
    RcclApi api;
    api.handle = h;
    api.get_unique_id = (decltype(api.get_unique_id))dlsym(h, "ncclGetUniqueId");
    api.comm_init_rank = (decltype(api.comm_init_rank))dlsym(h, "ncclCommInitRank");
    api.comm_destroy = (decltype(api.comm_destroy))dlsym(h, "ncclCommDestroy");
    api.all_reduce = (decltype(api.all_reduce))dlsym(h, "ncclAllReduce");
    api.error_string = (decltype(api.error_string))dlsym(h, "ncclGetErrorString");
    if (!api.get_unique_id || !api.comm_init_rank || !api.comm_destroy || !api.all_reduce || !api.error_string)
        return fail(VQHIP_ERCCL, "vqhip_rccl_load: librccl.so lacks an nccl* symbol");
    g_rccl = api;
    return VQHIP_OK;
}

int vqhip_rccl_unique_id(void *id_host) {
    if (!id_host) return fail(VQHIP_EINVAL, "vqhip_rccl_unique_id: null buffer");
    if (!g_rccl.handle) return fail(VQHIP_ERCCL, "vqhip_rccl_unique_id: call vqhip_rccl_load first");
    static_assert(sizeof(VqRcclId) == 128, "ncclUniqueId is 128 bytes (rccl.h: NCCL_UNIQUE_ID_BYTES)");
    const int rc = g_rccl.get_unique_id(id_host);
    return rc == 0 ? VQHIP_OK : rccl_fail("ncclGetUniqueId", rc);
}

int vqhip_rccl_comm_init(void **comm, int nranks, const void *id_host, int rank) {
    if (!comm || !id_host || nranks < 1 || rank < 0 || rank >= nranks) return fail(VQHIP_EINVAL, "vqhip_rccl_comm_init: bad argument");
    if (!g_rccl.handle) return fail(VQHIP_ERCCL, "vqhip_rccl_comm_init: call vqhip_rccl_load first");
    VqRcclId id;
    memcpy(id.bytes, id_host, sizeof(id.bytes));
    *comm = nullptr;
    const int rc = g_rccl.comm_init_rank(comm, nranks, id, rank);
    return rc == 0 ? VQHIP_OK : rccl_fail("ncclCommInitRank", rc);
}

int vqhip_rccl_comm_destroy(void *comm) {
    if (!comm) return VQHIP_OK;
    if (!g_rccl.handle) return fail(VQHIP_ERCCL, "vqhip_rccl_comm_destroy: RCCL not loaded");
    const int rc = g_rccl.comm_destroy(comm);
    return rc == 0 ? VQHIP_OK : rccl_fail("ncclCommDestroy", rc);
}

int vqhip_allreduce_packed(float *buf, int64_t floats, void *comm, void *stream) {
    if (!buf || !comm || floats < 0) return fail(VQHIP_EINVAL, "vqhip_allreduce_packed: bad argument");
    if (!g_rccl.handle) return fail(VQHIP_ERCCL, "vqhip_allreduce_packed: RCCL not loaded");
    if (floats == 0) return VQHIP_OK;
    const int rc = g_rccl.all_reduce(buf, buf, (size_t)floats, kNcclFloat32, kNcclSum, comm, (hipStream_t)stream);
    return rc == 0 ? VQHIP_OK : rccl_fail("ncclAllReduce", rc);
}
// ... 36 lines not shown
```

### vector_quantization_amd/csrc/vqhip_kernels.h

```cpp
#pragma once
#include <hip/hip_runtime.h>
#include <stdint.h>

#include <type_traits>

#include "vqhip_layout.h"

typedef _Float16 half8 __attribute__((ext_vector_type(8)));
typedef float f32x16 __attribute__((ext_vector_type(16)));
typedef float f32x4 __attribute__((ext_vector_type(4)));
typedef unsigned long long u64;

#define VQ_METRIC_DOT 2
#define VQ_METRIC_SWAP 0x100
#define VQ_METRIC_BF16 0x4
#define VQ_IS_BF16(m) (((m) & VQ_METRIC_BF16) != 0)
#define VQ_IS_L2(m) (((m) & 3) == VQHIP_METRIC_L2)
#define VQ_IS_COS(m) (((m) & 3) == VQHIP_METRIC_COS)
#define VQ_SWAPPED(m) (((m) & VQ_METRIC_SWAP) != 0)

#define VQ_F16_MIN_NORMAL 6.103515625e-05f
#define VQ_U 5.9604644775390625e-08f

__device__ __forceinline__ float bf16_to_f32(uint16_t b) { return __uint_as_float(((uint32_t)b) << 16); }
// ... 108 lines not shown
#pragma unroll
    for (int off = 32; off >= 1; off >>= 1) p = p + __shfl_xor(p, off, 64);
    return p;
}
__device__ __forceinline__ float wave_max(float p) {
#pragma unroll
    for (int off = 32; off >= 1; off >>= 1) p = fmaxf(p, __shfl_xor(p, off, 64));
    return p;
}

__device__ __forceinline__ float cb_scale(const VqCbStats *st) {
    float m = __uint_as_float(st->maxabs_bits);
    if (!(m > 0.0f) || st->nonfinite) return 1.0f;
    int ex;
    (void)frexpf(m, &ex);
    int sh = 14 - ex;
    sh = sh > 100 ? 100 : (sh < -100 ? -100 : sh);
    return ldexpf(1.0f, sh);
}


__device__ __forceinline__ void atomic_max_filtered(uint32_t *p, uint32_t v) {
    if (v > __hip_atomic_load(p, __ATOMIC_RELAXED, __HIP_MEMORY_SCOPE_AGENT)) atomicMax(p, v);
}

__device__ __forceinline__ int mfma_row(int r, int h) { return (r & 3) + 8 * (r >> 2) + 4 * h; }

__device__ __forceinline__ uint32_t cb_folded_mark(uint32_t r2, uint32_t eh2, uint32_t e2, uint32_t nonfinite) {
    uint32_t h = r2 * 0x9E3779B1u;
    h = (h ^ (h >> 15)) + eh2 * 0x85EBCA77u;
    h = (h ^ (h >> 13)) + e2 * 0xC2B2AE3Du;
    h = (h ^ (h >> 16)) + nonfinite * 0x27D4EB2Fu;
    return h | 0x80000000u;
}
__device__ __forceinline__ VqCbStats cb_stats_view(const VqCbStats *st) {
    VqCbStats v = *st;
    const int lane = threadIdx.x & 63;
    const uint32_t *slot = (const uint32_t *)((const char *)st + 256 + (lane & (VQ_CB_SLOTS - 1)) * 128);
    uint32_t r = slot[0], h = slot[1], bad = slot[2];
#pragma unroll
    for (int off = VQ_CB_SLOTS / 2; off >= 1; off >>= 1) {
        const uint32_t r2 = __shfl_xor(r, off, 64), h2 = __shfl_xor(h, off, 64), b2 = __shfl_xor(bad, off, 64);
        r = r > r2 ? r : r2; h = h > h2 ? h : h2; bad |= b2;
    }
    if (v.folded != 0u && v.folded == cb_folded_mark(v.r2max_bits, v.eh2max_bits, v.e2max_bits, v.nonfinite)) return v;
    if (v.part2_n != 0u) {
        const f32x4 *part = (const f32x4 *)((const char *)st + v.part2_off);
        float pr = 0.0f, ph = 0.0f, pb = 0.0f, pe = 0.0f;
        for (uint32_t base = 0; base < v.part2_n; base += 512u) {
            f32x4 q[8];
#pragma unroll
            for (int u = 0; u < 8; ++u) {
                const uint32_t i = base + (uint32_t)lane + 64u * (uint32_t)u;
                q[u] = part[i < v.part2_n ? i : 0u];
            }
#pragma unroll
            for (int u = 0; u < 8; ++u) { pr = fmaxf(pr, q[u][0]); ph = fmaxf(ph, q[u][1]); pb = fmaxf(pb, q[u][2]); pe = fmaxf(pe, q[u][3]); }
        }
#pragma unroll
        for (int off = 32; off >= 1; off >>= 1) {
            pr = fmaxf(pr, __shfl_xor(pr, off, 64)); ph = fmaxf(ph, __shfl_xor(ph, off, 64));
            pb = fmaxf(pb, __shfl_xor(pb, off, 64)); pe = fmaxf(pe, __shfl_xor(pe, off, 64));
        }
        v.r2max_bits = __float_as_uint(pr); v.eh2max_bits = __float_as_uint(ph); v.e2max_bits = __float_as_uint(pe);
        v.nonfinite |= (pb > 0.0f || !(pr == pr) || !(ph == ph) || !(pe == pe)) ? 1u : 0u;
        return v;
    }
    v.r2max_bits = r; v.eh2max_bits = h; v.nonfinite |= bad;
    return v;
}

__device__ __forceinline__ void cb_stats_publish(const VqCbStats *st) {
    if (blockIdx.x != 0 || (threadIdx.x >> 6) != 0) return;
    if (st->part2_n == 0u || st->folded != 0u) return;
    const VqCbStats v = cb_stats_view(st);
    if ((threadIdx.x & 63) == 0) {
        VqCbStats *w = const_cast<VqCbStats *>(st);
        w->r2max_bits = v.r2max_bits; w->eh2max_bits = v.eh2max_bits; w->e2max_bits = v.e2max_bits; w->nonfinite = v.nonfinite;
        asm volatile("s_waitcnt vmcnt(0)" ::: "memory");
        w->folded = cb_folded_mark(v.r2max_bits, v.eh2max_bits, v.e2max_bits, v.nonfinite);
    }
}

#include "vqhip_prepare_kernels.h"
#include "vqhip_proposal_kernels.h"
#include "vqhip_refine_kernels.h"
#include "vqhip_proposal32_kernels.h"
#include "vqhip_exact_kernels.h"
#include "vqhip_stream_kernels.h"
#include "vqhip_update_kernels.h"
#include "vqhip_sort_kernels.h"
#include "vqhip_aux_kernels.h"
#include "vqhip_exchange_kernels.h"
#include "vqhip_step_kernels.h"
```

### vector_quantization_amd/csrc/vqhip_proposal_kernels.h

```cpp
#pragma once
struct Top2 { float v1, v2, v3; uint32_t c1, c2; };
__device__ __forceinline__ float row_margin(const VqCbStats *st, int Dp, int metric, float X2, float R2, float *bf16_part = nullptr);

struct VqDecideOut {
    int64_t *idx; int32_t *hist;
    int *rescan_list, *multi_list, *exact_list, *counters;
    u64 *keys; float *thr_out; int *rescan_cnt;
    int *arrive;
    const int *n_dev;
    const void *xrows; float *xh2_w, *rho2_w, *xn_w;
};
template <bool AGENT>
__device__ __forceinline__ void decide_rows(int64_t n, bool oob, const VqCbStats *st, int Dp, int metric, int nslices,
                                            const float *rec, const float *xh2, const float *rho2, int64_t Np,
                                            const VqDecideOut &o, int *wcount, int *wbase, const float *rece2 = nullptr);

__device__ __forceinline__ void top_insert(Top2 &t, float v, uint32_t c) {
    if (v > t.v1) { t.v3 = fmaxf(t.v3, t.v2); t.v2 = t.v1; t.c2 = t.c1; t.v1 = v; t.c1 = c; }
    else if (v > t.v2) { t.v3 = fmaxf(t.v3, t.v2); t.v2 = v; t.c2 = c; }
    else t.v3 = fmaxf(t.v3, v);
}

__device__ __forceinline__ void top_merge_lane(Top2 &t, int xor_mask) {
    Top2 o;
    o.v1 = __shfl_xor(t.v1, xor_mask, 64); o.v2 = __shfl_xor(t.v2, xor_mask, 64); o.v3 = __shfl_xor(t.v3, xor_mask, 64);
    o.c1 = __shfl_xor(t.c1, xor_mask, 64); o.c2 = __shfl_xor(t.c2, xor_mask, 64);
    if (o.c1 != 0xFFFFFFFFu) top_insert(t, o.v1, o.c1);
    if (o.c2 != 0xFFFFFFFFu) top_insert(t, o.v2, o.c2);
    t.v3 = fmaxf(t.v3, o.v3);
}

__device__ __forceinline__ int tile_row16(int e, int lane) { return 16 * (e >> 2) + 4 * (lane >> 4) + (e & 3); }

#ifndef VQ_D32_PLAIN_OCC
#define VQ_D32_PLAIN_OCC 2
#endif
template <int NSTEP, int TT, int WAVES, int TPS, int NBUF = 2, bool FILTER = false, bool NOAUX = false,
          bool GROUPS = false, int XD = 0>
__global__ __launch_bounds__(WAVES * 64, (FILTER && NSTEP <= 2) ? (GROUPS ? 4 : VQ_D32_PLAIN_OCC) : WAVES / 4) void coarse_kernel(
    const char *__restrict__ ximg, int64_t N, const char *__restrict__ frag, int64_t nstages, int nslices,
    float *__restrict__ rec, int64_t Np, const VqCbStats *__restrict__ cbst, const float *__restrict__ xh2,
    const float *__restrict__ rho2, int Dp, int metric, VqDecideOut dec, int pad_stage, int tpb) {
    extern __shared__ __attribute__((aligned(16))) char lds[];
    static_assert(NSTEP % 2 == 0, "16x16x32 layout: 32-dim k-steps");
    static_assert(!GROUPS || FILTER, "group records are a form of the filtered epilogue");
    constexpr bool GBRANCH = TT >= VQ_GROUP_BRANCH_MIN_TT;
    constexpr bool PIPE = (TPS % 2) == 0;
    constexpr bool PIPE_H = (TPS == 1) && (WAVES <= 4);
    static_assert(!(PIPE_H && (NOAUX || FILTER)), "half-tile ping-pong: plain large-D form only");
    constexpr int NS32 = NSTEP / 2;
    constexpr int NCH = TPS * NSTEP + VQ_AUX_CHUNKS(TPS);
    constexpr int STAGE_BYTES = NCH * VQ_CHUNK_BYTES;
    constexpr int NE = 8;
#ifndef VQ_SCALAR_WAVE
#define VQ_SCALAR_WAVE 1
#endif
    const int lane = threadIdx.x & 63;
    const int wave = (VQ_SCALAR_WAVE && NSTEP > 2) ? __builtin_amdgcn_readfirstlane((int)(threadIdx.x >> 6)) : (int)(threadIdx.x >> 6);
    const int64_t ntt = (N + 31) / 32 * 2;
    if (dec.n_dev != nullptr) {
        const int64_t nd = *dec.n_dev;
        N = nd < N ? nd : N;
        if ((int64_t)(blockIdx.x / nslices) * tpb * 16 >= N) return;
    }
    const bool wave_active = wave * TT < tpb;
    cb_stats_publish(cbst);
    const int sl = blockIdx.x % nslices;
    const int64_t tb = blockIdx.x / nslices;
    const int64_t st0 = (nstages * sl) / nslices, st1 = (nstages * (sl + 1)) / nslices;
  for (bool once = true; once; once = false) {

    half8 xf[TT][NS32];
    if constexpr (XD == 0) {
#pragma unroll
        for (int t = 0; t < TT; ++t) {
            int64_t tt = tb * tpb + wave * TT + t;
            tt = tt < ntt ? tt : ntt - 1;
            const char *src = ximg + tt * (int64_t)(NS32 * VQ_CHUNK_BYTES) + lane * 16;
#pragma unroll
            for (int s = 0; s < NS32; ++s) xf[t][s] = *(const half8 *)(src + s * VQ_CHUNK_BYTES);
        }
    } else {
        static_assert(XD == 1 && !FILTER && !GROUPS && !NOAUX && (NSTEP % 4) == 0, "token side in the prologue: bf16 rows, plain D % 64 == 0 forms");
        const int q4 = lane >> 4, r16 = lane & 15;
        constexpr int Dr = NS32 * 32;
        static_assert(NS32 == 8 && NBUF >= 4 && 2 * STAGE_BYTES >= WAVES * 16 * 528, "row tile: D = 256, staged behind stage 1");
        char *stg = lds + 2 * STAGE_BYTES + wave * (16 * 528);
        const int hr = lane >> 5, c32 = lane & 31;
#pragma unroll
        for (int t = 0; t < TT; ++t) {
            const int64_t tok0 = (tb * tpb + wave * TT + t) * 16;
#pragma unroll
            for (int i = 0; i < 8; ++i) {
                const int64_t tok = tok0 + 2 * i + hr;
                const int64_t trow = tok < N ? tok : N - 1;
                xf[t][i] = *(const half8 *)((const uint16_t *)dec.xrows + trow * Dr + 8 * c32);
            }
        }
        __builtin_amdgcn_sched_barrier(0);
#pragma unroll
        for (int t = 0; t < TT; ++t) {
#pragma unroll
            for (int i = 0; i < 8; ++i) *(half8 *)(stg + (2 * i + hr) * 528 + 16 * c32) = xf[t][i];
#pragma unroll
            for (int s = 0; s < NS32; ++s) xf[t][s] = *(const half8 *)(stg + r16 * 528 + 64 * s + 16 * q4);
        }
#pragma unroll
        for (int t = 0; t < TT; ++t) {
            const int64_t tok = (tb * tpb + wave * TT + t) * 16 + r16;
            [[maybe_unused]] const int64_t trow = tok < N ? tok : N - 1;
            const bool stats = sl == 0;
            float sh[2] = {0.0f, 0.0f}, sr[2] = {0.0f, 0.0f}, pn[2][8];
#pragma unroll
            for (int j = 0; j < 8; ++j) { pn[0][j] = 0.0f; pn[1][j] = 0.0f; }
#pragma unroll
            for (int s = 0; s < NS32; ++s) {
                float v[8];
                half8 f;
                typedef uint32_t u32x4 __attribute__((ext_vector_type(4)));
                typedef _Float16 half2v __attribute__((ext_vector_type(2)));
                typedef float float2v __attribute__((ext_vector_type(2)));
                const u32x4 bits = __builtin_bit_cast(u32x4, xf[t][s]);
#pragma unroll
                for (int j = 0; j < 4; ++j) {
                    const uint32_t lo = bits[j] << 16, hi = bits[j] & 0xFFFF0000u;
                    v[2 * j] = __uint_as_float(lo); v[2 * j + 1] = __uint_as_float(hi);
                    float2v c;
                    c[0] = (lo & 0x7FFFFFFFu) < 0x38800000u ? 0.0f : v[2 * j];
                    c[1] = (hi & 0x7FFFFFFFu) < 0x38800000u ? 0.0f : v[2 * j + 1];
                    const half2v h = __builtin_convertvector(c, half2v);
                    f[2 * j] = h[0]; f[2 * j + 1] = h[1];
                }
                if (stats) {
#pragma unroll
                    for (int j = 0; j < 8; ++j) {
                        const float b = (float)f[j], res = v[j] - b;
                        sh[s & 1] = fmaf(b, b, sh[s & 1]); sr[s & 1] = fmaf(res, res, sr[s & 1]);
                        pn[s & 1][j] = fmaf(v[j], v[j], pn[s & 1][j]);
                    }
                }
                xf[t][s] = f;
            }
            if (!stats) continue;
            float a = 0.0f, b = 0.0f;
#pragma unroll
            for (int g = 0; g < 8; ++g) {
                a += __shfl(sh[g >> 2], (g & 3) * 16 + r16, 64);
                b += __shfl(sr[g >> 2], (g & 3) * 16 + r16, 64);
            }
            float q[8];
#pragma unroll
            for (int j = 0; j < 8; ++j) q[j] = pn[0][j] + pn[1][j];
#pragma unroll
            for (int j = 0; j < 8; ++j) q[j] = q[j] + __shfl_xor(q[j], 32, 64);
#pragma unroll
            for (int j = 0; j < 8; ++j) q[j] = q[j] + __shfl_xor(q[j], 16, 64);
            float a0 = q[0] + q[4], a1 = q[1] + q[5], a2 = q[2] + q[6], a3 = q[3] + q[7];
            a0 = a0 + a2; a1 = a1 + a3;
            a0 = a0 + a1;
            if (sl == 0 && q4 == 0 && tok < N && wave * TT + t < tpb) { dec.xh2_w[tok] = a; dec.rho2_w[tok] = b; dec.xn_w[tok] = a0; }
        }
    }
    if constexpr (PIPE_H) {
#pragma unroll
        for (int t = 0; t < TT; ++t)
#pragma unroll
            for (int s = 0; s < NS32; ++s) {
                if (t >= TT / 2) asm volatile("" : "+a"(xf[t][s]));
                else asm volatile("" : "+v"(xf[t][s]));
            }
    }

    float b1[TT], b2[TT], th[TT], mg[TT];
    uint32_t t1[TT];
#pragma unroll
    for (int t = 0; t < TT; ++t) { b1[t] = -INFINITY; b2[t] = -INFINITY; th[t] = -INFINITY; mg[t] = INFINITY; t1[t] = 0; }
    static_assert(!FILTER || PIPE, "the filtered epilogue is written for the ping-pong form");
    float sc0 = 0.0f, sc1 = 0.0f, sc2 = 0.0f;
    if constexpr (FILTER) {
        const VqCbStats stv = cb_stats_view(cbst);
#pragma unroll
        for (int t = 0; t < TT; ++t) {
            int64_t tokn = (tb * tpb + wave * TT + t) * 16 + (lane & 15);
            tokn = tokn < N ? tokn : N - 1;
            const float m = row_margin(&stv, Dp, metric, xh2[tokn], rho2[tokn]);
            mg[t] = (m > 0.0f) ? m : INFINITY;
        }
    }

    auto issue_stage = [&](int64_t st, int buf) {
        const char *src = frag + st * (int64_t)STAGE_BYTES;
        char *dstb = lds + buf * STAGE_BYTES;
        for (int c = wave; c < NCH; c += WAVES)
            __builtin_amdgcn_global_load_lds(
                (const __attribute__((address_space(1))) void *)(src + c * VQ_CHUNK_BYTES + lane * 16),
                (__attribute__((address_space(3))) void *)(dstb + c * VQ_CHUNK_BYTES), 16, 0, 0);
    };

    constexpr int AHEAD = NBUF >= 3 ? 2 : 1;
#ifndef VQ_LAG_MIN_STAGES
#define VQ_LAG_MIN_STAGES 48
#endif
    const int lag = (NBUF >= 4 && wave >= WAVES / 2 && st1 - st0 >= VQ_LAG_MIN_STAGES) ? 1 : 0;
    if (st0 < st1) issue_stage(st0, 0);
    if (AHEAD >= 2 && st0 + 1 < st1) issue_stage(st0 + 1, 1);
    vq_dma_barrier();

    f32x4 accA[2][TT], accB[2][TT];
#pragma unroll
    for (int c = 0; c < 2; ++c)
#pragma unroll
        for (int t = 0; t < TT; ++t)
#pragma unroll
            for (int q = 0; q < 4; ++q)
                accB[c][t][q] = GROUPS ? -INFINITY : -3.0e38f;
    if constexpr (PIPE_H) {
#pragma unroll
        for (int t = 0; t < TT; ++t) accA[1][t] = f32x4{-3.0e38f, -3.0e38f, -3.0e38f, -3.0e38f};
    }

    for (int64_t it = st0; it < st1 + ((NBUF >= 4 && st1 - st0 >= VQ_LAG_MIN_STAGES) ? 1 : 0); ++it) {
        if (it + AHEAD < st1) issue_stage(it + AHEAD, (int)((it + AHEAD - st0) % NBUF));
        const int64_t st = it - lag;
        if (st < st0 || st >= st1 || !wave_active) { vq_dma_barrier(); continue; }
        const int buf = (int)((st - st0) % NBUF);
        const char *base = lds + buf * STAGE_BYTES;
        const char *aux = base + TPS * NSTEP * VQ_CHUNK_BYTES;
      auto run_stage = [&](auto with_aux_tag) __attribute__((always_inline)) {
        constexpr bool WITH_AUX = decltype(with_aux_tag)::value;
        if constexpr (PIPE_H) {
            constexpr int PFH = VQ_PIPEH_PF;
            constexpr int TOTALH = 4 * TT;
            const uint32_t tile = (uint32_t)st;
#pragma unroll
            for (int c = 0; c < 2; ++c) {
                const f32x4 a4 = *(const f32x4 *)(aux + (16 * c + 4 * (lane >> 4)) * 4);
                uint32_t old[TT];
#pragma unroll
                for (int t = 0; t < TT; ++t) { accA[c][t] = a4; old[t] = __float_as_uint(b1[t]); }
                half8 af[PFH + 1];
#pragma unroll
                for (int i = 0; i < PFH; ++i) af[i] = *(const half8 *)(base + (2 * i + c) * VQ_CHUNK_BYTES + lane * 16);
#pragma unroll
// ... 214 lines not shown
                    const int rti = (int)(T[i] % TPS);
                    const char *sb = frag + rst * (int64_t)STAGE_BYTES;
#pragma unroll
                    for (int ch = 0; ch < NSTEP; ++ch)
                        a[i][ch] = *(const half8 *)(sb + (rti * NSTEP + ch) * VQ_CHUNK_BYTES + lane * 16);
#pragma unroll
                    for (int c = 0; c < 2; ++c) {
                        if (NOAUX && rst != (int64_t)pad_stage) acc[i][c] = f32x4{0.0f, 0.0f, 0.0f, 0.0f};
                        else acc[i][c] = *(const f32x4 *)(sb + TPS * NSTEP * VQ_CHUNK_BYTES + (rti * 32 + 16 * c + 4 * (lane >> 4)) * 4);
                    }
                }
                u64 done = 0;
#pragma unroll
                for (int i = 0; i < RB; ++i) {
#pragma unroll
                    for (int ch = 0; ch < NSTEP; ++ch)
                        acc[i][ch & 1] = __builtin_amdgcn_mfma_f32_16x16x32_f16(a[i][ch], xf[t][ch >> 1], acc[i][ch & 1], 0, 0, 0);
                    float w1 = -INFINITY, w2 = -INFINITY;
#pragma unroll
                    for (int e = 0; e < NE; ++e) {
                        float v = __uint_as_float((__float_as_uint(acc[i][e >> 2][e & 3]) & 0xFFFFFFF0u) | (uint32_t)e);
                        w2 = __builtin_amdgcn_fmed3f(w1, w2, v);
                        w1 = vmax(w1, v);
                    }
                    const bool mine = need && t1[t] == T[i];
                    e1 = mine ? w1 : e1; e2 = mine ? w2 : e2;
                    done |= __ballot(mine);
                }
                todo &= ~done;
            }
            const float other = bound_up(b2[t]);
            if (need) { b1[t] = e1; b2[t] = fmaxf(other, e2); }
            else { b2[t] = fmaxf(other, bound_up(b1[t])); }
            ident[t] = need;
        }
    }

#pragma unroll
    for (int t = 0; t < TT; ++t) {
        Top2 r; r.v1 = r.v2 = r.v3 = -INFINITY; r.c1 = r.c2 = 0xFFFFFFFFu;
        {
            uint32_t bits = __float_as_uint(b1[t]);
            uint32_t code = t1[t] * 32u + (uint32_t)tile_row16((int)(bits & 7u), lane);
            if (ident[t] && b1[t] > -INFINITY) top_insert(r, b1[t], code);
            r.v3 = fmaxf(r.v3, b2[t]);
        }
        top_merge_lane(r, 16);
        top_merge_lane(r, 32);
        const int64_t tokn = (tb * tpb + wave * TT + t) * 16 + (lane & 15);
        if (lane < 16 && tokn < N && wave * TT + t < tpb) {
            float *rp = rec + (int64_t)sl * VQ_REC_FIELDS * Np + tokn;
            if (dec.idx != nullptr && nslices > 1) {
                __hip_atomic_store(rp, r.v1, __ATOMIC_RELAXED, __HIP_MEMORY_SCOPE_AGENT);
                __hip_atomic_store(rp + Np, __uint_as_float(r.c1), __ATOMIC_RELAXED, __HIP_MEMORY_SCOPE_AGENT);
                __hip_atomic_store(rp + 2 * Np, r.v2, __ATOMIC_RELAXED, __HIP_MEMORY_SCOPE_AGENT);
                __hip_atomic_store(rp + 3 * Np, __uint_as_float(r.c2), __ATOMIC_RELAXED, __HIP_MEMORY_SCOPE_AGENT);
                __hip_atomic_store(rp + 4 * Np, r.v3, __ATOMIC_RELAXED, __HIP_MEMORY_SCOPE_AGENT);
            } else {
                rp[0] = r.v1; rp[Np] = __uint_as_float(r.c1); rp[2 * Np] = r.v2;
                rp[3 * Np] = __uint_as_float(r.c2); rp[4 * Np] = r.v3;
            }
        }
    }

    if (dec.idx != nullptr) {
        int *flags = (int *)lds;
        asm volatile("s_waitcnt vmcnt(0)" ::: "memory");
        __syncthreads();
        if (threadIdx.x == 0) {
            int last = 1;
            if (nslices > 1) {
                last = (atomicAdd(&dec.arrive[tb], 1) == nslices - 1) ? 1 : 0;
            }
            flags[0] = last;
        }
        __syncthreads();
        const bool last = flags[0] != 0;
        __syncthreads();
        if (last) {
            int *wcount = (int *)lds, *wbase = wcount + 3 * 16;
            int64_t n = tb * (int64_t)(tpb * 16) + threadIdx.x;
            const bool oob = (int)threadIdx.x >= tpb * 16 || n >= N;
            if (n >= N) n = N - 1;
            decide_rows<true>(n, oob, cbst, Dp, metric, nslices, rec, xh2, rho2, Np, dec, wcount, wbase);
        }
    }
  }
}
```

### vector_quantization_amd/csrc/vqhip_refine_kernels.h

```cpp
#pragma once
template <int DT>
__device__ float sqnorm_thread(const void *x, int64_t off, int D) {
    float p[64];
#pragma unroll
    for (int j = 0; j < 64; ++j) p[j] = 0.0f;
    for (int base = 0; base < D; base += 64) {
#pragma unroll
        for (int j = 0; j < 64; ++j)
            if (base + j < D) { float a = load_elem<DT>(x, off + base + j); p[j] = fmaf(a, a, p[j]); }
    }
#pragma unroll
    for (int off2 = 32; off2 >= 1; off2 >>= 1)
#pragma unroll
        for (int j = 0; j < 32; ++j)
            if (j < off2) p[j] = p[j] + p[j + off2];
    return p[0];
}

template <int DT>
__device__ float oracle_distance(const void *x, int64_t xoff, const float *erow, int D, int metric, float xn, float en) {
    float c = 0.0f;
    if (VQ_IS_L2(metric)) {
        for (int d = 0; d < D; ++d) c = fmaf(-2.0f * load_elem<DT>(x, xoff + d), erow[d], c);
        float t = (c + xn) + en;
        t = (t < 0.0f) ? 0.0f : t;
        return sqrtf(t);
    }
    for (int d = 0; d < D; ++d) c = fmaf(load_elem<DT>(x, xoff + d), erow[d], c);
    return cos_distance(c, metric);
}

__device__ __forceinline__ u64 dist_key(float d, uint32_t k) {
    if (isnan(d)) return (u64)k;
    if (d == 0.0f) d = 0.0f;
    uint32_t b = __float_as_uint(d);
    b = (b & 0x80000000u) ? ~b : (b | 0x80000000u);
    return ((u64)b + 1ull) << 32 | (u64)k;
}

__device__ __forceinline__ float row_margin(const VqCbStats *st, int Dp, int metric, float X2, float R2, float *bf16_part) {
    if (bf16_part) *bf16_part = 0.0f;
    if (st->nonfinite != 0 || !isfinite(X2) || !isfinite(R2)) return -1.0f;
    const float infl = 1.0f + 1e-5f;
    float se = cb_scale(st);
    float Xh = sqrtf(X2) * infl, rho = sqrtf(R2) * infl, Xn = Xh + rho;
    float Emax = sqrtf(__uint_as_float(st->e2max_bits)) * infl;
    float Rmax = sqrtf(__uint_as_float(st->r2max_bits)) * infl;
    float Ehmax = sqrtf(__uint_as_float(st->eh2max_bits)) * infl;
    float ENmax = __uint_as_float(st->enmax_bits);
    float Df = (float)Dp;
    float m;
    if (VQ_IS_L2(metric)) {
        float mag = Xn * Xn + ENmax + 2.0f * Xn * Emax;
        if (!(mag < 1e30f)) return -1.0f;
        float S = 2.0f * (1.01f * Df * VQ_U * 2.0f * Xn * Emax + 2.1f * VQ_U * mag) + 4.0f * VQ_U * mag;
        float B = rho * Emax + Xh * Rmax + (4.0f * Df + 32.0f) * VQ_U * (Xh * Ehmax + 0.5f * ENmax);
        m = 2.0f * B + 0.5f * S;
        if (st->l2_const_norm != 0) m += __uint_as_float(st->en_spread_bits);
    } else {
        float B = rho * Emax + Xh * Rmax + (4.0f * Df + 32.0f) * VQ_U * (Xh * Ehmax);
        m = 2.0f * B + 2.0f * (Df + 4.0f) * VQ_U * Xn * Emax + 8.0f * VQ_U;
        if (VQ_IS_BF16(metric)) {
            const float wworst = 3.0f * 0.0078125f * 1.01f * fmaxf(1.0f, Xn * Emax);
            m += wworst;
            if (bf16_part) *bf16_part = wworst * se * infl;
        }
    }
    m = m * se * infl + 1e-37f;
    if (!isfinite(m)) { if (bf16_part) *bf16_part = 0.0f; return -1.0f; }
    return m;
}

#define VQ_RESCAN_CAP 32
#ifndef VQ_RESCAN_LOCAL
#define VQ_RESCAN_LOCAL 8
#endif

template <bool AGENT>
__device__ __forceinline__ float rec_load(const float *p) {
    if constexpr (AGENT) return __hip_atomic_load(p, __ATOMIC_RELAXED, __HIP_MEMORY_SCOPE_AGENT);
    else return *p;
}

__device__ __forceinline__ float bf16_tight_margin(float m, float bf16_worst, float gbest, const VqCbStats *st) {
    if (!(bf16_worst > 0.0f) || !(m > 0.0f) || !isfinite(gbest)) return m;
    const float se = cb_scale(st);
    const float s = gbest / se, err = (m - bf16_worst) / se;
    const float spread = 1.0f + 2.0f * (fmaxf(err, 0.0f) + fmaxf(-s, 0.0f) + fmaxf(s - 1.0f, 0.0f));
    const float width = 0.0078125f * 1.02f * spread * se * 1.0001f;
    return width < bf16_worst ? m - bf16_worst + width : m;
}

template <int NSL, bool AGENT, bool GROUPS = false>
__device__ __forceinline__ void decide_rows_impl(int64_t n, bool oob, const VqCbStats *st, int Dp, int metric, int nslices,
                                                 const float *rec, const float *xh2, const float *rho2, int64_t Np,
                                                 const VqDecideOut &o, int *wcount, int *wbase, const float *rece2 = nullptr) {
    const VqCbStats stv = cb_stats_view(st);
    float bf16_worst = 0.0f;
    float m = row_margin(&stv, Dp, metric, xh2[n], rho2[n], &bf16_worst);
    bool invalid = !(m > 0.0f);
    float gbest = -INFINITY;
    int nc = 0;
    bool unidentified = false;
    uint32_t best = 0xFFFFFFFFu;
    float thr;
    if constexpr (NSL > 0) {
        float v1[NSL], v2[NSL], v3[NSL], c1[NSL], c2[NSL];
#pragma unroll
        for (int s = 0; s < NSL; ++s) {
            const float *rp = rec + (int64_t)s * VQ_REC_FIELDS * Np + n;
            v1[s] = rec_load<AGENT>(rp); c1[s] = rec_load<AGENT>(rp + Np);
            v2[s] = rec_load<AGENT>(rp + 2 * Np); v3[s] = rec_load<AGENT>(rp + 4 * Np);
            if constexpr (GROUPS) {
                c2[s] = rec_load<AGENT>(rp + 3 * Np);
                v3[s] = fmaxf(v3[s], fmaxf(rece2[(int64_t)(2 * s) * Np + n], rece2[(int64_t)(2 * s + 1) * Np + n]));
            }
        }
#pragma unroll
        for (int s = 0; s < NSL; ++s) gbest = fmaxf(gbest, GROUPS ? fmaxf(v1[s], v2[s]) : v1[s]);
        if (!(gbest > -INFINITY) || !isfinite(gbest)) invalid = true;
        m = bf16_tight_margin(m, bf16_worst, gbest, &stv);
        thr = gbest - m;
#pragma unroll
        for (int s = 0; s < NSL; ++s) {
            if (v3[s] >= thr) unidentified = true;
            if (v1[s] >= thr) { ++nc; best = __float_as_uint(c1[s]); }
            if (v2[s] >= thr) { ++nc; if constexpr (GROUPS) best = __float_as_uint(c2[s]); }
        }
    } else {
        static_assert(!GROUPS, "the group path runs with 1, 2 or 4 slices");
        for (int s = 0; s < nslices; ++s) gbest = fmaxf(gbest, rec_load<AGENT>(rec + (int64_t)s * VQ_REC_FIELDS * Np + n));
        if (!(gbest > -INFINITY) || !isfinite(gbest)) invalid = true;
        m = bf16_tight_margin(m, bf16_worst, gbest, &stv);
        thr = gbest - m;
        for (int s = 0; s < nslices; ++s) {
            const float *rp = rec + (int64_t)s * VQ_REC_FIELDS * Np + n;
            const float v1 = rec_load<AGENT>(rp), v2 = rec_load<AGENT>(rp + 2 * Np), v3 = rec_load<AGENT>(rp + 4 * Np);
            if (v3 >= thr) unidentified = true;
            if (v1 >= thr) { ++nc; best = __float_as_uint(rec_load<AGENT>(rp + Np)); }
            if (v2 >= thr) ++nc;
        }
    }
    const int lane = threadIdx.x & 63, wave = threadIdx.x >> 6;
    const bool to_exact = !oob && (invalid || nc == 0);
    const bool to_rescan = !oob && !to_exact && unidentified;
    const bool to_multi = !oob && !to_exact && !to_rescan && nc > 1;
    const u64 mk_e = __ballot(to_exact), mk_r = __ballot(to_rescan), mk_m = __ballot(to_multi);
    if (lane == 0) { wcount[0 * 16 + wave] = __popcll(mk_r); wcount[1 * 16 + wave] = __popcll(mk_m); wcount[2 * 16 + wave] = __popcll(mk_e); }
    __syncthreads();
    if (threadIdx.x < 3) {
        int tot = 0;
        const int nw = blockDim.x >> 6;
        for (int i = 0; i < nw; ++i) { wbase[threadIdx.x * 16 + i] = tot; tot += wcount[threadIdx.x * 16 + i]; }
        const int base = tot ? atomicAdd(&o.counters[threadIdx.x], tot) : 0;
        for (int i = 0; i < nw; ++i) wbase[threadIdx.x * 16 + i] += base;
    }
    __syncthreads();
    const u64 below = (1ull << lane) - 1ull;
    if (to_exact) { o.exact_list[wbase[2 * 16 + wave] + __popcll(mk_e & below)] = (int)n; o.keys[n] = ~0ull; }
    if (to_rescan) { int pos = wbase[0 * 16 + wave] + __popcll(mk_r & below); o.rescan_list[pos] = (int)n; o.rescan_cnt[pos] = 0; o.thr_out[n] = thr; }
    if (to_multi) o.multi_list[wbase[1 * 16 + wave] + __popcll(mk_m & below)] = (int)n;
    if (oob) return;
    if (!to_exact && !to_rescan && !to_multi) {
        o.idx[n] = (int64_t)best;
        if (o.hist) atomicAdd(&o.hist[best], 1);
    }
}

template <bool AGENT>
__device__ __forceinline__ void decide_rows(int64_t n, bool oob, const VqCbStats *st, int Dp, int metric, int nslices,
                                            const float *rec, const float *xh2, const float *rho2, int64_t Np,
                                            const VqDecideOut &o, int *wcount, int *wbase, const float *rece2) {
    if (rece2 != nullptr) {
        switch (nslices) {
#define VQ_DECIDE_CASE(NSL) case NSL: decide_rows_impl<NSL, AGENT, true>(n, oob, st, Dp, metric, nslices, rec, xh2, rho2, Np, o, wcount, wbase, rece2); break;
            VQ_DECIDE_CASE(1) VQ_DECIDE_CASE(2) VQ_DECIDE_CASE(4)
#undef VQ_DECIDE_CASE
            default: break;
        }
        return;
    }
    switch (nslices) {
#define VQ_DECIDE_CASE(NSL) case NSL: decide_rows_impl<NSL, AGENT>(n, oob, st, Dp, metric, nslices, rec, xh2, rho2, Np, o, wcount, wbase); break;
        VQ_DECIDE_CASE(1) VQ_DECIDE_CASE(2) VQ_DECIDE_CASE(4) VQ_DECIDE_CASE(8) VQ_DECIDE_CASE(16)
#undef VQ_DECIDE_CASE
        default: decide_rows_impl<0, AGENT>(n, oob, st, Dp, metric, nslices, rec, xh2, rho2, Np, o, wcount, wbase); break;
    }
}

__global__ void refine_decide_kernel(const char *cb, VqCbLayout L, int64_t N, int metric, int nslices, const float *rec,
                                     const float *xh2, const float *rho2, int64_t Np, VqDecideOut o, const float *rece2 = nullptr) {
    __shared__ int wcount[3 * 16];
    __shared__ int wbase[3 * 16];
    if (o.n_dev != nullptr) {
        const int64_t nd = *o.n_dev;
        N = nd < N ? nd : N;
        if ((int64_t)blockIdx.x * blockDim.x >= N) return;
    }
    int64_t n = (int64_t)blockIdx.x * blockDim.x + threadIdx.x;
    const bool oob = n >= N;
    if (oob) n = N - 1;
    decide_rows<false>(n, oob, (const VqCbStats *)(cb + L.off_stats), L.Dp, metric, nslices, rec, xh2, rho2, Np, o, wcount, wbase, rece2);
}

template <int NSTEP, int TT, int WAVES, int TPS, int NBUF = 2, int XD = 0>
__global__ __launch_bounds__(WAVES * 64) void rescan_kernel(const char *__restrict__ ximg, const char *__restrict__ frag,
                                                            int64_t nstages, const int *__restrict__ rescan_list,
                                                            const int *__restrict__ counters, const float *__restrict__ thr,
                                                            int *__restrict__ rescan_cnt, int *__restrict__ cand_list,
                                                            const void *__restrict__ xrows = nullptr) {
    extern __shared__ __attribute__((aligned(16))) char lds[];
    constexpr int NS32 = NSTEP / 2;
    constexpr int NCH = TPS * NSTEP + VQ_AUX_CHUNKS(TPS);
    constexpr int STAGE_BYTES = NCH * VQ_CHUNK_BYTES;
    constexpr int BM = WAVES * TT * 16;
    constexpr int PF = NSTEP <= 32 ? 1 : (NSTEP <= 48 ? 2 : 4);
    int *lcnt = (int *)(lds + NBUF * STAGE_BYTES);
    uint32_t *lcand = (uint32_t *)(lds + NBUF * STAGE_BYTES) + BM;
    constexpr int AHEAD = NBUF >= 4 ? 2 : 1;
    const int lane = threadIdx.x & 63, wave = threadIdx.x >> 6;
    const int nrows = counters[0];
    if (nrows <= 0) return;
    const int64_t ntb = (nrows + BM - 1) / BM;
    int64_t ns = 1;
    while (ntb * ns * 2 <= (int64_t)gridDim.x && ns * 2 <= nstages) ns <<= 1;

    auto issue_stage = [&](int64_t st, int buf) {
        const char *src = frag + st * (int64_t)STAGE_BYTES;
        char *dstb = lds + buf * STAGE_BYTES;
        for (int c = wave; c < NCH; c += WAVES)
            __builtin_amdgcn_global_load_lds(
                (const __attribute__((address_space(1))) void *)(src + c * VQ_CHUNK_BYTES + lane * 16),
                (__attribute__((address_space(3))) void *)(dstb + c * VQ_CHUNK_BYTES), 16, 0, 0);
    };

    for (int64_t item = blockIdx.x; item < ntb * ns; item += gridDim.x) {
        const int64_t sl = item % ns, tb = item / ns;
        const int64_t st0 = (nstages * sl) / ns, st1 = (nstages * (sl + 1)) / ns;
        issue_stage(st0, 0);
        if (AHEAD >= 2 && st0 + 1 < st1) issue_stage(st0 + 1, 1);
        for (int i = threadIdx.x; i < BM; i += WAVES * 64) lcnt[i] = 0;
        half8 xf[TT][NS32];
        float mythr[TT];
        int slot[TT];
#pragma unroll
        for (int t = 0; t < TT; ++t) {
            int64_t tt = tb * (BM / 16) + wave * TT + t;
            slot[t] = (int)(tt * 16 + (lane & 15));
            const bool valid = slot[t] < nrows;
            const int64_t tk = rescan_list[valid ? slot[t] : nrows - 1];
            mythr[t] = valid ? thr[tk] : INFINITY;
            if constexpr (XD == 0) {
                const char *src = ximg + (tk >> 4) * (int64_t)(NS32 * VQ_CHUNK_BYTES) + ((lane >> 4) * 16 + (int)(tk & 15)) * 16;
#pragma unroll
                for (int s = 0; s < NS32; ++s) xf[t][s] = *(const half8 *)(src + s * VQ_CHUNK_BYTES);
            } else {
#pragma unroll
                for (int s = 0; s < NS32; ++s) {
                    float v[8];
                    load8<1>(xrows, tk * (int64_t)(NS32 * 32) + 32 * s + 8 * (lane >> 4), v);
                    half8 f;
#pragma unroll
                    for (int j = 0; j < 8; ++j) f[j] = to_f16_ftz(v[j]);
                    xf[t][s] = f;
                }
            }
        }
        vq_dma_barrier();
        for (int64_t st = st0; st < st1; ++st) {
// ... 253 lines not shown
```

### vector_quantization_amd/csrc/vqhip_update_kernels.h

```cpp
#pragma once
__device__ __forceinline__ void nt_store4(float *q, float a, float b, float c, float d) {
    __builtin_nontemporal_store(a, q); __builtin_nontemporal_store(b, q + 1);
    __builtin_nontemporal_store(c, q + 2); __builtin_nontemporal_store(d, q + 3);
}

template <int DT, int NT>
__global__ __launch_bounds__(1024) void gather_ste_loss_kernel(const void *x, const float *e, const int64_t *idx, int64_t N,
                                                              int D, float *z, float *zste, double *sse,
                                                              float *mse = nullptr, float beta = 0.0f) {
    __shared__ double red[16];
    const int lane = threadIdx.x & 63, wave = threadIdx.x >> 6;
    double s = 0.0;
    const bool vec = (D % 4) == 0;
    const int64_t stride = (int64_t)gridDim.x * 16;
    int64_t n = (int64_t)blockIdx.x * 16 + wave;
    for (; n < N; n += stride) {
        const float *er = e + idx[n] * D;
        if (vec) {
            for (int d = lane * 4; d < D; d += 256) {
                float4 zv = *(const float4 *)(er + d);
                float xv[4];
                if (DT == 0) {
                    float4 t = *(const float4 *)((const float *)x + n * D + d);
                    xv[0] = t.x; xv[1] = t.y; xv[2] = t.z; xv[3] = t.w;
                } else {
                    const uint32_t *px = (const uint32_t *)((const uint16_t *)x + n * D + d);
                    uint2 t;
                    if (NT) { t.x = __builtin_nontemporal_load(px); t.y = __builtin_nontemporal_load(px + 1); }
                    else t = *(const uint2 *)px;
                    xv[0] = __uint_as_float(t.x << 16); xv[1] = __uint_as_float(t.x & 0xFFFF0000u);
                    xv[2] = __uint_as_float(t.y << 16); xv[3] = __uint_as_float(t.y & 0xFFFF0000u);
                }
                float d0 = zv.x - xv[0], d1 = zv.y - xv[1], d2 = zv.z - xv[2], d3 = zv.w - xv[3];
                if (NT) {
                    if (z) nt_store4(z + n * D + d, zv.x, zv.y, zv.z, zv.w);
                    if (zste) nt_store4(zste + n * D + d, xv[0] + d0, xv[1] + d1, xv[2] + d2, xv[3] + d3);
                } else {
                    if (z) *(float4 *)(z + n * D + d) = zv;
                    if (zste) *(float4 *)(zste + n * D + d) = make_float4(xv[0] + d0, xv[1] + d1, xv[2] + d2, xv[3] + d3);
                }
                s += (double)((d0 * d0 + d1 * d1) + (d2 * d2 + d3 * d3));
            }
        } else {
            for (int d = lane; d < D; d += 64) {
                float xv = load_elem<DT>(x, n * D + d), zv = er[d];
                float df = zv - xv;
                if (z) z[n * D + d] = zv;
                if (zste) zste[n * D + d] = xv + df;
                s += (double)(df * df);
            }
        }
    }
    if (sse) {
#pragma unroll
        for (int off = 32; off >= 1; off >>= 1) s += __shfl_xor(s, off, 64);
        if (lane == 0) red[wave] = s;
        __syncthreads();
        if (threadIdx.x == 0) {
            double t = 0.0;
#pragma unroll
            for (int i = 0; i < 16; ++i) t += red[i];
            if (!mse) {
                atomicAdd(sse, t);
            } else {
                int *ticket = (int *)(sse + 1);
                const double before = atomicAdd(sse, t);
                asm volatile("" :: "v"(before) : "memory");
                if (atomicAdd(ticket, 1) == (int)gridDim.x - 1) {
                    const double total = __hip_atomic_load(sse, __ATOMIC_RELAXED, __HIP_MEMORY_SCOPE_AGENT);
                    const float mean = (float)(total / ((double)N * (double)D));
                    mse[0] = mean; mse[1] = mean;
                    const float weighted = beta * mean;
                    mse[2] = mean + weighted; mse[3] = 0.0f;
                    __hip_atomic_store(sse, 0.0, __ATOMIC_RELAXED, __HIP_MEMORY_SCOPE_AGENT);
                    __hip_atomic_store(ticket, 0, __ATOMIC_RELAXED, __HIP_MEMORY_SCOPE_AGENT);
                }
            }
        }
    }
}

template <int DT>
__global__ __launch_bounds__(256) void gather_ste_map_kernel(const void *__restrict__ x, const float *__restrict__ e,
                                                             const int64_t *__restrict__ idx, int64_t N, int D, int64_t hw,
                                                             float *__restrict__ out_map, double *sse, float *mse, float beta) {
    __shared__ float tile[64][65];
    __shared__ double red[4];
    __shared__ int64_t code_s[64];
    const int lane = threadIdx.x & 63, wave = threadIdx.x >> 6;
    double s = 0.0;
    const int64_t ntiles = (N + 63) / 64;
    const bool vec = (D % 4) == 0 && (hw % 4) == 0;
    for (int64_t tb = blockIdx.x; tb < ntiles; tb += gridDim.x) {
        const int64_t n0 = tb * 64;
        __syncthreads();
        if (threadIdx.x < 64) code_s[threadIdx.x] = (n0 + threadIdx.x < N) ? idx[n0 + threadIdx.x] : 0;
        __syncthreads();
        if (vec) {
            const int cl = 4 * (lane & 15);
            const int t4 = 4 * (lane & 15);
            const int64_t nw = n0 + t4;
            const int64_t wbase = (nw < N) ? ((nw / hw) * (int64_t)D * hw + (nw % hw)) : 0;
            float4 zc[4], zn[4];
            typename std::conditional<DT == 0, float4, uint2>::type xc[4], xnx[4];
            auto load_chunk = [&](int c0, float4 (&zr)[4], decltype(xc) &xr) {
#pragma unroll
                for (int i = 0; i < 4; ++i) {
                    const int tl = 16 * i + 4 * wave + (lane >> 4);
                    const int64_t n = n0 + tl;
                    if (n < N && c0 + cl < D) {
                        zr[i] = *(const float4 *)(e + code_s[tl] * D + c0 + cl);
                        if (x != nullptr) {
                            if constexpr (DT == 0) xr[i] = *(const float4 *)((const float *)x + n * D + c0 + cl);
                            else xr[i] = *(const uint2 *)((const uint16_t *)x + n * D + c0 + cl);
                        }
                    }
                }
            };
            load_chunk(0, zc, xc);
            for (int c0 = 0; c0 < D; c0 += 64) {
                if (c0 + 64 < D) load_chunk(c0 + 64, zn, xnx);
#pragma unroll
                for (int i = 0; i < 4; ++i) {
                    const int tl = 16 * i + 4 * wave + (lane >> 4);
                    const int64_t n = n0 + tl;
                    float o[4] = {0.0f, 0.0f, 0.0f, 0.0f};
                    if (n < N && c0 + cl < D) {
                        const float4 zv = zc[i];
                        if (x != nullptr) {
                            float xv[4];
                            if constexpr (DT == 0) { xv[0] = xc[i].x; xv[1] = xc[i].y; xv[2] = xc[i].z; xv[3] = xc[i].w; }
                            else {
                                xv[0] = __uint_as_float(xc[i].x << 16); xv[1] = __uint_as_float(xc[i].x & 0xFFFF0000u);
                                xv[2] = __uint_as_float(xc[i].y << 16); xv[3] = __uint_as_float(xc[i].y & 0xFFFF0000u);
                            }
                            const float d0 = zv.x - xv[0], d1 = zv.y - xv[1], d2 = zv.z - xv[2], d3 = zv.w - xv[3];
                            s += (double)((d0 * d0 + d1 * d1) + (d2 * d2 + d3 * d3));
                            o[0] = xv[0] + d0; o[1] = xv[1] + d1; o[2] = xv[2] + d2; o[3] = xv[3] + d3;
                        } else {
                            o[0] = zv.x; o[1] = zv.y; o[2] = zv.z; o[3] = zv.w;
                        }
                    }
#pragma unroll
                    for (int j = 0; j < 4; ++j) tile[cl + j][tl] = o[j];
                }
                __syncthreads();
#pragma unroll
                for (int i = 0; i < 4; ++i) {
                    const int dl = 16 * i + 4 * wave + (lane >> 4);
                    if (c0 + dl < D && nw < N) {
                        float *dst = out_map + wbase + (int64_t)(c0 + dl) * hw;
                        if (nw + 3 < N) *(float4 *)dst = make_float4(tile[dl][t4], tile[dl][t4 + 1], tile[dl][t4 + 2], tile[dl][t4 + 3]);
                        else
                            for (int j = 0; j < 4 && nw + j < N; ++j) dst[j] = tile[dl][t4 + j];
                    }
                }
                __syncthreads();
#pragma unroll
                for (int i = 0; i < 4; ++i) { zc[i] = zn[i]; xc[i] = xnx[i]; }
            }
// ... 380 lines not shown
```

### vector_quantization_amd/quantizers/vector_quantizer.py

```python
from __future__ import annotations

import os
from typing import Optional

import torch
from torch import nn

from .. import functional as VF
from .. import ops, train_step
from ..config import Config, Item, RegistryMeta
from ..registries import InitRegistry, ModelRegistry, VQITQuantizerDistanceRegistry, VQITQuantizerRegistry
from .memo import Memo, get_memo
from .quantizer_api import BaseQuantizer
from .callbacks import CVQVAECallback, NormalizeCallback, VQKDCallback
from .distances import BaseDistance, CosineDistance, L2Distance, LazyDistance
from .losses import CodebookLoss, CommitmentLoss, VQGANLoss


@VQITQuantizerRegistry.register_()
class VectorQuantizer(BaseQuantizer):
    one_call_steps = os.environ.get('VQHIP_ONE_CALL', '1') != '0'

    def __init__(self, *args, embedding: nn.Embedding, distance: BaseDistance, fused: bool = True,
                 cache_codebook: bool = False, **kwargs) -> None:
# ... 97 lines not shown

    def _fusable(self) -> bool:
        if not self._fused or self._callbacks.overrides_decode_or_loss():
            return False
        if type(self)._decode is not VectorQuantizer._decode or type(self)._loss is not BaseQuantizer._loss:
            return False
        for loss in self._losses.values():
            if not (isinstance(loss, (VQGANLoss, CodebookLoss, CommitmentLoss)) and loss.plain):
                return False
        return True

    def _vqgan_beta(self) -> float:
        return next((loss.beta for loss in self._losses.values() if isinstance(loss, VQGANLoss)), 0.0)

    def _loss_values(self, memo: Memo, m_cb, m_cm, m_vqgan, beta: float, like: torch.Tensor) -> torch.Tensor:
        losses = {}
        for name, loss in self._losses.items():
            if isinstance(loss, VQGANLoss):
                losses[name] = m_vqgan if loss.beta == beta else torch.add(m_cb, m_cm, alpha=loss.beta)
            elif isinstance(loss, CodebookLoss):
                losses[name] = m_cb
            else:
                losses[name] = m_cm
        loss_memo = get_memo(memo, 'loss')
        loss_memo.update(losses)
        memo['loss'] = loss_memo
        values = list(losses.values())
        if len(values) == 1:
            return values[0]
        return sum(values, like.new_zeros([], dtype=torch.float32))

    def _one_call_step(self, x: torch.Tensor):
        if not (self.one_call_steps and self._fused and x.dim() == 2):
            return None
        cbs = self._callbacks.callbacks
        if len(cbs) > 1 or type(self)._encode is not VectorQuantizer._encode or type(self)._decode is not VectorQuantizer._decode \
                or type(self)._loss is not BaseQuantizer._loss or type(self).encode is not BaseQuantizer.encode:
            return None
        if len(cbs) == 0 or type(cbs[0]) is NormalizeCallback:
            w = self._embedding.weight
            ok = (self._fusable() and not self._cache_codebook and type(self._distance) in (L2Distance, CosineDistance)
                  and x.is_cuda and 0 < x.shape[0] < (1 << 31) and w.is_cuda and w.dtype == torch.float32 and w.is_contiguous())
            return self._forward_plain if ok else None
        if not self.training:
            return None
        cb = cbs[0]
        if type(cb) is CVQVAECallback:
            return self._forward_cvq if (self._fusable() and cb.fused_forward_ok(x)) else None
        if type(cb) is VQKDCallback:
            losses = list(self._losses.values())
            ok = (len(losses) == 1 and type(losses[0]) is CommitmentLoss and losses[0]._mse.norm
                  and losses[0]._mse._weight._value == 1.0 and losses[0]._weight._value == 1.0)
            return self._forward_vqkd if (ok and cb.fused_forward_ok(x)) else None
        return None

    def _encode_memo(self, memo: Memo, out: dict, x_op: torch.Tensor, e_op: torch.Tensor) -> None:
        enc = get_memo(memo, 'encode')
        prepared = out['prepared']
        if out['xq'] is not None:
            xq, eq = out['xq'], prepared.exact_rows()
        else:
            xq, eq = (out['xn'] if out.get('xn') is not None else out['x']), prepared.weight
        enc['distance'] = LazyDistance(self._distance, x_op, e_op, xq=xq, eq=eq, metric=ops.metric_name(prepared.metric))
        if out['hist'] is not None:
            enc['hist'] = out['hist']
        memo['encode'] = enc

    def _forward_cvq(self, x: torch.Tensor, memo: Memo):
        beta = self._vqgan_beta()
        quant, z_ste, m_cb, m_cm, m_vqgan = self._callbacks.callbacks[0].fused_forward(x, memo, beta)
        memo.update(x=x, quant=quant)
        memo['decode'] = get_memo(memo, 'decode')
        return z_ste, self._loss_values(memo, m_cb, m_cm, m_vqgan, beta, x), memo

    def _forward_plain(self, x: torch.Tensor, memo: Memo):
        cbs = self._callbacks.callbacks
        weight = self._embedding.weight
        normalize = len(cbs) == 1
        w_in = weight.detach()
        w_out = None
        if normalize:
            w_out = w_in if cbs[0]._writes_in_place(weight) else torch.empty_like(w_in)
        beta = self._vqgan_beta()
        out = train_step.vq_forward(x.detach(), w_in, w_out, self._distance.metric_for(weight.shape[1]), beta, normalize=normalize,
                                    want_hist=self.training and len(cbs) > 0)
        if normalize:
            cbs[0]._publish_weight(weight, w_out)
        done = VF._Computed(xn=out['xn'], z_ste=out['z_ste'], mse=out['mse'], idx=out['idx'])
        xn, z_ste, m_cb, m_cm, m_vqgan = VF.vq_step(x, weight, done, beta)
        rows = xn if normalize else x
        grad = torch.is_grad_enabled() and (x.requires_grad or weight.requires_grad)
        self._encode_memo(memo, out, rows if grad else (out['xn'] if normalize else out['x']),
                          weight.view_as(weight) if (grad and weight.requires_grad) else out['prepared'].weight)
        memo.update(x=rows, quant=out['idx'])
        memo['decode'] = get_memo(memo, 'decode')
        return z_ste, self._loss_values(memo, m_cb, m_cm, m_vqgan, beta, x), memo

    def _forward_vqkd(self, x: torch.Tensor, memo: Memo):
        cb = self._callbacks.callbacks[0]
        xn, quant, z_ste, value = cb.fused_forward(x, memo)
        memo.update(x=xn, quant=quant)
        memo['decode'] = get_memo(memo, 'decode')
        loss_memo = get_memo(memo, 'loss')
        loss_memo.update({next(iter(self._losses.keys())): value})
        memo['loss'] = loss_memo
        return z_ste, value, memo

    def forward(self, x: torch.Tensor, memo: Memo) -> tuple[torch.Tensor, torch.Tensor, Memo]:
        step = self._one_call_step(x)
        if step is not None:
            return step(x, memo)
        if not self._fusable() or x.dim() != 2:
            z, loss, memo = super().forward(x, memo)
            z = VF.ste(z, memo['x'])
            return z, loss, memo
        x, quant, memo = self.encode(x, memo)
        memo.update(x=x, quant=quant)
        beta = self._vqgan_beta()
        z_ste, m_cb, m_cm, m_vqgan = VF.fused_decode_loss(x, self._embedding.weight, quant, beta)
        memo['decode'] = get_memo(memo, 'decode')
        return z_ste, self._loss_values(memo, m_cb, m_cm, m_vqgan, beta, x), memo


    def map_fusable(self, x: torch.Tensor) -> bool:
        from .callbacks import BaseCallback
        if not (x.dim() == 4 and x.is_cuda and x.is_contiguous() and x.dtype in (torch.float32, torch.bfloat16)):
            return False
        if x.shape[1] != self.embedding_dim or not ops.coarse_supported(x.shape[1]) or x.data_ptr() % 16 or self._cache_codebook:
            return False
        if type(self)._encode is not VectorQuantizer._encode or not hasattr(self._distance, 'encode_map'):
            return False
        if len(self._forward_pre_hooks) > 0 or len(self._forward_hooks) > 0:
            return False
        return all(type(cb).before_encode is BaseCallback.before_encode for cb in self._callbacks.callbacks)

    def encode_map(self, x_map: torch.Tensor, memo: Memo) -> tuple[torch.Tensor, torch.Tensor, Memo]:
        enc = get_memo(memo, 'encode')
        w = self._embedding.weight.detach()
        hist = None
        if self.training and len(self._callbacks.callbacks) > 0:
            hist = torch.empty(self.codebook_size, dtype=torch.int32, device=x_map.device)
        stash = {}
        quant, x_rows = self._distance.encode_map(x_map, w, hist=hist, stash=stash, zero_hist=True)
        enc['distance'] = LazyDistance(self._distance, x_rows, w, xq=stash.get('xq'), eq=stash.get('eq'), metric=stash.get('metric'))
        if hist is not None:
            enc['hist'] = hist
        memo['encode'] = enc
        return x_rows, self._callbacks.after_encode(x_rows, quant, memo), memo

    def forward_map(self, x_map: torch.Tensor, memo: Memo) -> tuple[torch.Tensor, torch.Tensor, Memo]:
        assert self.map_fusable(x_map) and self._fusable()
        x_rows, quant, memo = self.encode_map(x_map, memo)
        memo.update(x=x_rows, quant=quant)
        beta = self._vqgan_beta()
        z_map, m_cb, m_cm, m_vqgan = VF.fused_map_decode_loss(x_map, x_rows, self._embedding.weight, quant, beta)
        memo['decode'] = get_memo(memo, 'decode')
        loss = self._loss_values(memo, m_cb, m_cm, m_vqgan, beta, x_map)
        return z_map, loss, memo

    def decode_map(self, quant: torch.Tensor, memo: Memo) -> tuple[torch.Tensor, Memo]:
        b, h, w = quant.shape
        z_map, _ = ops.gather_ste_map(None, self._embedding.weight.detach(), quant.reshape(-1), b, h, w)
        return z_map, memo


@VQITQuantizerRegistry.register_()
class VQGANQuantizer(VectorQuantizer):

# ... 12 lines not shown
```

### vector_quantization_amd/train_step.py

```python
from __future__ import annotations

import ctypes
import os
import time
from typing import Optional

import torch

from . import _lib, ops
from ._lib import STEP_AFTER_EXCHANGE, STEP_ALL, STEP_BEFORE_EXCHANGE, STEP_PACK_SYNC, check
from .ops import METRICS, _bytes, _codebook, _latents, _mse_scratch, _on_tensor_device, _stream


def _p(t: Optional[torch.Tensor]):
    return t.data_ptr() if t is not None else None


class _Arena:

    def __init__(self) -> None:
        self._bufs: dict = {}

    def get(self, key, ws_bytes: int, packed_floats: int, device):
        if torch.cuda.is_current_stream_capturing():
# ... 144 lines not shown
    a.count_event = (state.event_handle or None) if (use_host_word and not capturing) else None
    a.comm = comm
    a.packed, a.packed_floats = _p(packed), (packed.numel() if packed is not None else 0)
    a.ws, a.ws_bytes = ws.data_ptr(), ws.numel()
    a.cap_used, a.exchange_floats = -1, 0
    a.early_word_host = state.early_host.data_ptr() if early_count else None
    a.early_seq_dev = state.seq_dev.data_ptr() if early_count else None
    sync = bool(anchor_sync and exchange)
    a.anchor_sync, a.rank = int(sync), int(rank)
    keys = None
    if sync:
        if capturing:
            keys = torch.empty(K, dtype=torch.int64, device=dev)
        else:
            if state.keys is None:
                state.keys = torch.empty(K, dtype=torch.int64, device=dev)
            keys = state.keys
    a.keys = _p(keys)
    if cap < 0 and not state.event_handle:
        a.cap = state.wait_count()
    between = ()
    if _caller_exchanges(exchange, comm, world, all_reduce):
        between = (lambda: all_reduce(packed[:a.exchange_floats]),)
        if sync:
            between = (lambda: a.cap_used > 0 and all_reduce_min(keys[:a.cap_used]),) + between
    _run(L.vqhip_cvq_forward, 'vqhip_cvq_forward', a, between)
    if use_host_word and prefetch and not capturing and not state.event_handle:
        state.event.record()
    out.update(prepared=ops.PreparedCodebook(image, w_in, K, D, m), cap_used=int(a.cap_used), exchange_floats=int(a.exchange_floats))
    return out


class VqkdStepState:

    def __init__(self) -> None:
        self.arena = _Arena()


@_on_tensor_device
def vqkd_forward(x: torch.Tensor, w_in: torch.Tensor, w_mid: torch.Tensor, w_out: torch.Tensor, metric, ema_decay: float,
                 state: VqkdStepState, *, exchange: bool, world: int, comm: Optional[int], all_reduce=None,
                 ordered: bool = False, tail: bool = True):
    ops._require_cuda(x, w_in, w_mid, w_out)
    L = _lib.lib()
    a = _lib.VqkdForwardArgs()
    out, image, (N, K, D, dt, m) = _begin(a, x, w_in, metric, xq=True, tail=tail)
    dev = out['x'].device
    floats = ops.pack_floats(K, K, D)
    ws, packed = state.arena.get((N, K, D, dt), L.vqhip_vqkd_forward_ws_bytes(N, K, D), floats, dev)
    xn = torch.empty(N, D, dtype=torch.float32, device=dev)
    a.world = int(world)
    a.ema_decay = float(ema_decay)
    a.exchange, a.ordered, a.tail = int(bool(exchange)), int(bool(ordered)), int(bool(tail))
    a.w_mid, a.w_out = w_mid.data_ptr(), w_out.data_ptr()
    a.xn = xn.data_ptr()
    a.comm = comm
    a.packed, a.packed_floats = packed.data_ptr(), packed.numel()
    a.ws, a.ws_bytes = ws.data_ptr(), ws.numel()
    _run(L.vqhip_vqkd_forward, 'vqhip_vqkd_forward', a,
         (lambda: all_reduce(packed[:floats]),) if _caller_exchanges(exchange, comm, world, all_reduce) else ())
    out.update(xn=xn, prepared=ops.PreparedCodebook(image, w_mid, K, D, m))
    return out


@_on_tensor_device
def vq_forward(x: torch.Tensor, w_in: torch.Tensor, w_out: Optional[torch.Tensor], metric, beta: float, *, normalize: bool,
               want_hist: bool, tail: bool = True):
    ops._require_cuda(x, w_in)
    L = _lib.lib()
    a = _lib.VqForwardArgs()
    out, image, (N, K, D, dt, m) = _begin(a, x, w_in, metric, hist=want_hist, tail=tail)
    dev = out['x'].device
    ws = _bytes(L.vqhip_workspace_bytes(N, K, D), dev)
    xn = torch.empty(N, D, dtype=torch.float32, device=dev) if normalize else None
    a.normalize, a.beta = int(bool(normalize)), float(beta)
    a.w_out, a.xn = _p(w_out), _p(xn)
    a.ws, a.ws_bytes = ws.data_ptr(), ws.numel()
    check(L.vqhip_vq_forward(ctypes.byref(a), _stream()), 'vqhip_vq_forward')
    out.update(xn=xn, prepared=ops.PreparedCodebook(image, w_out if normalize else w_in, K, D, m))
    return out


@_on_tensor_device
def vqkd_backward(x: torch.Tensor, xn: torch.Tensor, w: torch.Tensor, idx: torch.Tensor, g_zste: Optional[torch.Tensor],
                  g_loss: Optional[torch.Tensor]) -> torch.Tensor:
    ops._require_cuda(x, xn, w, idx)
    x, dt = _latents(x)
    N, D = x.shape
    w = _codebook(w)
    gx = torch.empty(N, D, dtype=torch.float32, device=x.device)
    if g_zste is not None:
        g_zste = g_zste.float().contiguous()
    if g_loss is not None:
        g_loss = g_loss.detach().float().reshape(1).contiguous()
    check(_lib.lib().vqhip_vqkd_backward(x.data_ptr(), dt, xn.data_ptr(), w.data_ptr(), idx.data_ptr(), N, D, _p(g_zste), _p(g_loss),
                                         gx.data_ptr(), _stream()), 'vqhip_vqkd_backward')
    return gx
```

Before: 160.4 million tokens/s.

## Fuse gather/STE/MSE decode into the argmin decide stage for eval forward

```diff
diff --git a/include/vqhip.h b/include/vqhip.h
--- a/include/vqhip.h
+++ b/include/vqhip.h
@@ -210,6 +210,10 @@
 } vqhip_vq_forward_t;
 int vqhip_vq_forward(vqhip_vq_forward_t *args, void *stream);
 
+int vqhip_vq_eval_forward(const void *x, int x_dtype, const float *e, int64_t N, int64_t K, int D, int metric, void *cb, int64_t cb_bytes,
+                          int64_t *idx, float *xq, float *z, float *z_ste, float *mse, float beta, void *scratch16, void *ws,
+                          int64_t ws_bytes, void *stream);
+
 int vqhip_gather_rows(const void *x, int x_dtype, const int64_t *row_idx, int64_t K, int D, float *out,
                       void *stream);
 
diff --git a/vector_quantization_amd/_lib.py b/vector_quantization_amd/_lib.py
--- a/vector_quantization_amd/_lib.py
+++ b/vector_quantization_amd/_lib.py
@@ -83,6 +83,7 @@
     'vqhip_normalize_rows': (_i32, [_vp, _i32, _i64, _i32, _f32, _vp, _vp]),
     'vqhip_gather_ste_loss': (_i32, [_vp, _i32, _vp, _vp, _i64, _i32, _vp, _vp, _vp, _vp]),
     'vqhip_gather_ste_mse': (_i32, [_vp, _i32, _vp, _vp, _i64, _i32, _vp, _vp, _vp, _f32, _vp, _vp]),
+    'vqhip_vq_eval_forward': (_i32, [_vp, _i32, _vp, _i64, _i64, _i32, _i32, _vp, _i64, _vp, _vp, _vp, _vp, _vp, _f32, _vp, _vp, _i64, _vp]),
     'vqhip_hist': (_i32, [_vp, _i64, _i64, _vp, _vp]),
     'vqhip_hist_i32': (_i32, [_vp, _i64, _i64, _vp, _vp]),
     'vqhip_fsq_encode': (_i32, [ctypes.POINTER(FsqConstants), _vp, _i32, _i32, _i64, _i64, _vp, _vp, _i32, _vp, _vp, _vp]),
diff --git a/vector_quantization_amd/csrc/vqhip.hip b/vector_quantization_amd/csrc/vqhip.hip
--- a/vector_quantization_amd/csrc/vqhip.hip
+++ b/vector_quantization_amd/csrc/vqhip.hip
@@ -86,6 +86,7 @@
 static std::atomic<int> g_tune_slices{0};
 static std::atomic<int> g_tune_force_exact{0};
 static std::atomic<int> g_tune_stream{1};
+static std::atomic<int> g_tune_unfused{0};
 #define VQ_FUSED_DECIDE_MAX_N 16384
 
 template <int NSTEP, int TT, int WAVES, int TPS, int NBUF = 2, bool FILTER = false, bool NOAUX = false, bool GROUPS = false, int XD = 0>
@@ -160,6 +161,7 @@
     return best;
 }
 
+#define VQ_XD_BLOCK_ROWS (8 * 4 * 16)
 static bool vq_xdirect(int64_t N, int64_t K, int D, int x_dtype, int metric, const int *n_dev) {
     if (D != 256 || n_dev != nullptr || vq_cb_layout(K, D).nstages < 2 || g_tune_slices.load() == 1) return false;
     if (x_dtype != VQHIP_DTYPE_BF16) return false;
@@ -196,7 +198,7 @@
         *nslices_out = ns;                                                                          \
         const int tpb = (ns == 1) ? balanced_tiles_per_block(N, (W) * (TT)) : (W) * (TT);           \
         VqDecideOut dsel = dec;                                                                     \
-        if (!(ns == 1 || N <= VQ_FUSED_DECIDE_MAX_N)) dsel.idx = nullptr;                           \
+        if (!(ns == 1 || N <= VQ_FUSED_DECIDE_MAX_N || dec.sse != nullptr)) dsel.idx = nullptr;     \
         *fused_decide_out = dsel.idx != nullptr ? 1 : 0;                                            \
         return launch_coarse_cfg<NS, TT, W, __VA_ARGS__>(ximg, N, frag, L.nstages, ns, rec, Np, cbst, xh2, rho2, L.Dp, metric, dsel, pad_stage, tpb, s); \
     }
@@ -441,9 +443,10 @@
 int vqhip_argmin_exact(const void *x, int x_dtype, const float *e, int64_t N, int64_t K, int D, int metric, int64_t *idx,
                        float *dmin, int32_t *hist, void *ws, int64_t ws_bytes, void *stream);
 
+struct VqFusedDecode { const float *e; float *z, *z_ste; double *sse; float *mse; float beta; bool done; };
 static int argmin_pipeline(const void *x, int x_dtype, const float *e_exact, const void *cb, int64_t N, int64_t K, int D,
                            int metric, int64_t *idx, int32_t *hist, void *ws, void *stream, bool x_prepared = false,
-                           const int *n_dev = nullptr) {
+                           const int *n_dev = nullptr, VqFusedDecode *fd = nullptr) {
     hipStream_t s = (hipStream_t)stream;
     VqCbLayout L = vq_cb_layout(K, D);
     VqWsLayout W = vq_ws_layout(N, K, D);
@@ -474,6 +477,9 @@
     }
     VqDecideOut dec{idx, hist, rescan_list, multi_list, exact_list, counters, keys, thr, rescan_cnt, arrive, n_dev,
                     x, xh2, rho2, (float *)(w + W.off_xn)};
+    const bool fuse = fd != nullptr && xd;
+    const int fuse_nt = fuse && (int64_t)N * D * 4 * ((fd->z ? 1 : 0) + (fd->z_ste ? 1 : 0)) > (192ll << 20);
+    if (fuse) { dec.e_dec = fd->e; dec.zste_dec = fd->z_ste; dec.z_dec = fd->z; dec.sse = fd->sse; dec.nt_dec = fuse_nt; }
     VqDecideOut dec_arg = dec;
     int fused_done = 0;
     VqGroupLists grp{nullptr, nullptr, nullptr, nullptr, 0, 1, 0};
@@ -538,7 +544,18 @@
         force_exact_rows_kernel<<<1, 1024, 0, s>>>((int)(force < N ? force : N), exact_list, counters, keys);
         VQ_CHECK_LAUNCH("force_exact_rows_kernel");
     }
-    return run_exact_rows(x, x_dtype, e_exact, en, xnorm, N, K, D, metric, exact_list, counters + 2, keys, counters + 3, idx, hist, s);
+    rc = run_exact_rows(x, x_dtype, e_exact, en, xnorm, N, K, D, metric, exact_list, counters + 2, keys, counters + 3, idx, hist, s);
+    if (rc || !fuse) return rc;
+    {
+        const int64_t want = (N + 255) / 256;
+        const int grid = (int)(want > 512 ? 512 : want);
+        const int nprop = (int)((N + VQ_XD_BLOCK_ROWS - 1) / VQ_XD_BLOCK_ROWS);
+        if (fuse_nt) decode_listed_kernel<1><<<grid, 1024, 0, s>>>(x, fd->e, idx, N, rescan_list, multi_list, exact_list, counters, rescan_cnt, fd->z, fd->z_ste, fd->sse, fd->mse, fd->beta, nprop);
+        else decode_listed_kernel<0><<<grid, 1024, 0, s>>>(x, fd->e, idx, N, rescan_list, multi_list, exact_list, counters, rescan_cnt, fd->z, fd->z_ste, fd->sse, fd->mse, fd->beta, nprop);
+        VQ_CHECK_LAUNCH("decode_listed_kernel");
+        fd->done = true;
+    }
+    return VQHIP_OK;
 }
 
 static int encode_fused_front(const void *rows, int rows_dtype, int64_t N, const float *codes, int64_t Kc, int D, int cb_metric,
@@ -584,8 +601,16 @@
     return vqhip_encode_ex(x, x_dtype, e, N, K, D, metric, cb, cb_bytes, idx, hist, xq, ws, ws_bytes, 0, stream);
 }
 
+static int encode_impl(const void *x, int x_dtype, const float *e, int64_t N, int64_t K, int D, int metric, void *cb, int64_t cb_bytes,
+                       int64_t *idx, int32_t *hist, float *xq, void *ws, int64_t ws_bytes, int flags, void *stream, VqFusedDecode *fd);
+
 int vqhip_encode_ex(const void *x, int x_dtype, const float *e, int64_t N, int64_t K, int D, int metric, void *cb, int64_t cb_bytes,
                     int64_t *idx, int32_t *hist, float *xq, void *ws, int64_t ws_bytes, int flags, void *stream) {
+    return encode_impl(x, x_dtype, e, N, K, D, metric, cb, cb_bytes, idx, hist, xq, ws, ws_bytes, flags, stream, nullptr);
+}
+
+static int encode_impl(const void *x, int x_dtype, const float *e, int64_t N, int64_t K, int D, int metric, void *cb, int64_t cb_bytes,
+                       int64_t *idx, int32_t *hist, float *xq, void *ws, int64_t ws_bytes, int flags, void *stream, VqFusedDecode *fd) {
     const bool zero_hist = hist != nullptr && (flags & VQHIP_ENCODE_ZERO_HIST) != 0;
     if (N == 0 || !vq_coarse_supported(D)) {
         if (zero_hist && K > 0) VQ_HIP(hipMemsetAsync(hist, 0, (size_t)K * 4, (hipStream_t)stream));
@@ -614,7 +639,7 @@
     VqCbLayout L = vq_cb_layout(K, D);
     const float *e_exact = cos ? (const float *)((const char *)cb + L.off_eexact) : e;
     return argmin_pipeline(cos ? (const void *)xq : x, cos ? VQHIP_DTYPE_F32 : x_dtype, e_exact, cb, N, K, D, metric, idx, hist, ws,
-                           stream, true);
+                           stream, true, nullptr, cos ? nullptr : fd);
 }
 
 int vqhip_encode_map(const void *x_map, int x_dtype, const float *e, int64_t B, int64_t HW, int64_t K, int D, int metric, void *cb,
@@ -1513,6 +1538,18 @@
     return VQHIP_OK;
 }
 
+int vqhip_vq_eval_forward(const void *x, int x_dtype, const float *e, int64_t N, int64_t K, int D, int metric, void *cb, int64_t cb_bytes,
+                          int64_t *idx, float *xq, float *z, float *z_ste, float *mse, float beta, void *scratch16, void *ws,
+                          int64_t ws_bytes, void *stream) {
+    if (!mse || !scratch16 || N <= 0) return fail(VQHIP_EINVAL, "vqhip_vq_eval_forward: bad argument");
+    VqFusedDecode fd{e, z, z_ste, (double *)scratch16, mse, beta, false};
+    const bool fused = metric == VQHIP_METRIC_L2 && (z || z_ste) && !g_tune_unfused.load() && !g_tune_force_exact.load() &&
+                       vq_xdirect(N, K, D, x_dtype, metric, nullptr);
+    if (int rc = encode_impl(x, x_dtype, e, N, K, D, metric, cb, cb_bytes, idx, nullptr, xq, ws, ws_bytes, 0, stream, fused ? &fd : nullptr)) return rc;
+    if (fd.done) return VQHIP_OK;
+    return vqhip_gather_ste_mse(x, x_dtype, e, idx, N, D, z, z_ste, mse, beta, scratch16, stream);
+}
+
 int vqhip_vqkd_backward(const void *x, int x_dtype, const float *xn, const float *w, const int64_t *idx, int64_t N, int D,
                         const float *g_zste, const float *g_loss, float *grad_x, void *stream) {
     if (!x || !xn || !w || !idx || !grad_x || N < 0 || D <= 0) return fail(VQHIP_EINVAL, "vqhip_vqkd_backward: bad argument");
@@ -1738,6 +1775,7 @@
 int vqhip_set_tuning(int key, int value) {
     if (key == 2) g_tune_slices = (value == 1 || value == 2 || value == 4 || value == 8 || value == 16) ? value : 0;
     else if (key == 18) g_tune_stream = value != 0;
+    else if (key == 20) g_tune_unfused = value != 0;
     else if (key == 12) g_tune_force_exact = value > 0 ? (value < 1024 ? value : 1024) : 0;
     else return fail(VQHIP_EINVAL, "vqhip_set_tuning: unknown key");
     return VQHIP_OK;
diff --git a/vector_quantization_amd/csrc/vqhip_kernels.h b/vector_quantization_amd/csrc/vqhip_kernels.h
--- a/vector_quantization_amd/csrc/vqhip_kernels.h
+++ b/vector_quantization_amd/csrc/vqhip_kernels.h
@@ -214,6 +214,36 @@
     }
 }
 
+__device__ __forceinline__ void nt_store4(float *q, float a, float b, float c, float d) {
+    __builtin_nontemporal_store(a, q); __builtin_nontemporal_store(b, q + 1);
+    __builtin_nontemporal_store(c, q + 2); __builtin_nontemporal_store(d, q + 3);
+}
+
+template <int NT>
+__device__ __forceinline__ uint2 row256_load_bf16(const void *x, int64_t n, int lane) {
+    const uint32_t *px = (const uint32_t *)((const uint16_t *)x + n * 256 + lane * 4);
+    uint2 t;
+    if (NT) { t.x = __builtin_nontemporal_load(px); t.y = __builtin_nontemporal_load(px + 1); }
+    else t = *(const uint2 *)px;
+    return t;
+}
+template <int NT>
+__device__ __forceinline__ float row256_decode(uint2 t, float4 zv, float *z, float *zste, int64_t n, int lane) {
+    float xv[4];
+    xv[0] = __uint_as_float(t.x << 16); xv[1] = __uint_as_float(t.x & 0xFFFF0000u);
+    xv[2] = __uint_as_float(t.y << 16); xv[3] = __uint_as_float(t.y & 0xFFFF0000u);
+    const float d0 = zv.x - xv[0], d1 = zv.y - xv[1], d2 = zv.z - xv[2], d3 = zv.w - xv[3];
+    const int64_t o = n * 256 + lane * 4;
+    if (NT) {
+        if (z) nt_store4(z + o, zv.x, zv.y, zv.z, zv.w);
+        if (zste) nt_store4(zste + o, xv[0] + d0, xv[1] + d1, xv[2] + d2, xv[3] + d3);
+    } else {
+        if (z) *(float4 *)(z + o) = zv;
+        if (zste) *(float4 *)(zste + o) = make_float4(xv[0] + d0, xv[1] + d1, xv[2] + d2, xv[3] + d3);
+    }
+    return (d0 * d0 + d1 * d1) + (d2 * d2 + d3 * d3);
+}
+
 #include "vqhip_prepare_kernels.h"
 #include "vqhip_proposal_kernels.h"
 #include "vqhip_refine_kernels.h"
diff --git a/vector_quantization_amd/csrc/vqhip_proposal_kernels.h b/vector_quantization_amd/csrc/vqhip_proposal_kernels.h
--- a/vector_quantization_amd/csrc/vqhip_proposal_kernels.h
+++ b/vector_quantization_amd/csrc/vqhip_proposal_kernels.h
@@ -9,11 +9,13 @@
     int *arrive;
     const int *n_dev;
     const void *xrows; float *xh2_w, *rho2_w, *xn_w;
+    const float *e_dec; float *zste_dec, *z_dec; double *sse; int nt_dec;
 };
-template <bool AGENT>
+template <bool AGENT, bool ASTATS = false>
 __device__ __forceinline__ void decide_rows(int64_t n, bool oob, const VqCbStats *st, int Dp, int metric, int nslices,
                                             const float *rec, const float *xh2, const float *rho2, int64_t Np,
-                                            const VqDecideOut &o, int *wcount, int *wbase, const float *rece2 = nullptr);
+                                            const VqDecideOut &o, int *wcount, int *wbase, const float *rece2 = nullptr,
+                                            int *settled = nullptr);
 
 __device__ __forceinline__ void top_insert(Top2 &t, float v, uint32_t c) {
     if (v > t.v1) { t.v3 = fmaxf(t.v3, t.v2); t.v2 = t.v1; t.c2 = t.c1; t.v1 = v; t.c1 = c; }
@@ -31,6 +33,30 @@
 }
 
 __device__ __forceinline__ int tile_row16(int e, int lane) { return 16 * (e >> 2) + 4 * (lane >> 4) + (e & 3); }
+
+template <int NT, int WAVES>
+__device__ __forceinline__ double decode_settled(const VqDecideOut &dec, const int *settled, int64_t n0, int nrows, int wave, int lane) {
+    constexpr int RB = 8;
+    double s = 0.0;
+    for (int r0 = wave * RB; r0 < nrows; r0 += WAVES * RB) {
+        int code[RB];
+        uint2 xb[RB];
+        float4 zv[RB];
+#pragma unroll
+        for (int i = 0; i < RB; ++i) code[i] = __builtin_amdgcn_readfirstlane(settled[r0 + i]);
+#pragma unroll
+        for (int i = 0; i < RB; ++i) {
+            if (code[i] >= 0) {
+                xb[i] = row256_load_bf16<NT>(dec.xrows, n0 + r0 + i, lane);
+                zv[i] = *(const float4 *)(dec.e_dec + (int64_t)code[i] * 256 + lane * 4);
+            }
+        }
+#pragma unroll
+        for (int i = 0; i < RB; ++i)
+            if (code[i] >= 0) s += (double)row256_decode<NT>(xb[i], zv[i], dec.z_dec, dec.zste_dec, n0 + r0 + i, lane);
+    }
+    return s;
+}
 
 #ifndef VQ_D32_PLAIN_OCC
 #define VQ_D32_PLAIN_OCC 2
@@ -158,7 +184,13 @@
             float a0 = q[0] + q[4], a1 = q[1] + q[5], a2 = q[2] + q[6], a3 = q[3] + q[7];
             a0 = a0 + a2; a1 = a1 + a3;
             a0 = a0 + a1;
-            if (sl == 0 && q4 == 0 && tok < N && wave * TT + t < tpb) { dec.xh2_w[tok] = a; dec.rho2_w[tok] = b; dec.xn_w[tok] = a0; }
+            if (sl == 0 && q4 == 0 && tok < N && wave * TT + t < tpb) {
+                if (dec.idx != nullptr) {
+                    __hip_atomic_store(dec.xh2_w + tok, a, __ATOMIC_RELAXED, __HIP_MEMORY_SCOPE_AGENT);
+                    __hip_atomic_store(dec.rho2_w + tok, b, __ATOMIC_RELAXED, __HIP_MEMORY_SCOPE_AGENT);
+                    __hip_atomic_store(dec.xn_w + tok, a0, __ATOMIC_RELAXED, __HIP_MEMORY_SCOPE_AGENT);
+                } else { dec.xh2_w[tok] = a; dec.rho2_w[tok] = b; dec.xn_w[tok] = a0; }
+            }
         }
     }
     if constexpr (PIPE_H) {
@@ -539,7 +571,30 @@
             int64_t n = tb * (int64_t)(tpb * 16) + threadIdx.x;
             const bool oob = (int)threadIdx.x >= tpb * 16 || n >= N;
             if (n >= N) n = N - 1;
-            decide_rows<true>(n, oob, cbst, Dp, metric, nslices, rec, xh2, rho2, Np, dec, wcount, wbase);
+            if constexpr (XD == 1) {
+                int *settled = (int *)lds + 128;
+                decide_rows<true, true>(n, oob, cbst, Dp, metric, nslices, rec, xh2, rho2, Np, dec, wcount, wbase, nullptr, settled);
+                if (dec.sse != nullptr) {
+                    __syncthreads();
+                    double s = dec.nt_dec ? decode_settled<1, WAVES>(dec, settled, tb * (int64_t)(tpb * 16), tpb * 16, wave, lane)
+                                          : decode_settled<0, WAVES>(dec, settled, tb * (int64_t)(tpb * 16), tpb * 16, wave, lane);
+#pragma unroll
+                    for (int off = 32; off >= 1; off >>= 1) s += __shfl_xor(s, off, 64);
+                    double *red = (double *)(lds + 4096);
+                    if (lane == 0) red[wave] = s;
+                    __syncthreads();
+                    if (threadIdx.x == 0) {
+                        double t = 0.0;
+#pragma unroll
+                        for (int i = 0; i < WAVES; ++i) t += red[i];
+                        const double before = atomicAdd(dec.sse, t);
+                        asm volatile("" :: "v"(before) : "memory");
+                        atomicAdd((int *)(dec.sse + 1), 1);
+                    }
+                }
+            } else {
+                decide_rows<true>(n, oob, cbst, Dp, metric, nslices, rec, xh2, rho2, Np, dec, wcount, wbase);
+            }
         }
     }
   }
diff --git a/vector_quantization_amd/csrc/vqhip_refine_kernels.h b/vector_quantization_amd/csrc/vqhip_refine_kernels.h
--- a/vector_quantization_amd/csrc/vqhip_refine_kernels.h
+++ b/vector_quantization_amd/csrc/vqhip_refine_kernels.h
@@ -91,13 +91,14 @@
     return width < bf16_worst ? m - bf16_worst + width : m;
 }
 
-template <int NSL, bool AGENT, bool GROUPS = false>
+template <int NSL, bool AGENT, bool GROUPS = false, bool ASTATS = false>
 __device__ __forceinline__ void decide_rows_impl(int64_t n, bool oob, const VqCbStats *st, int Dp, int metric, int nslices,
                                                  const float *rec, const float *xh2, const float *rho2, int64_t Np,
-                                                 const VqDecideOut &o, int *wcount, int *wbase, const float *rece2 = nullptr) {
+                                                 const VqDecideOut &o, int *wcount, int *wbase, const float *rece2 = nullptr,
+                                                 int *settled = nullptr) {
     const VqCbStats stv = cb_stats_view(st);
     float bf16_worst = 0.0f;
-    float m = row_margin(&stv, Dp, metric, xh2[n], rho2[n], &bf16_worst);
+    float m = row_margin(&stv, Dp, metric, rec_load<ASTATS>(xh2 + n), rec_load<ASTATS>(rho2 + n), &bf16_worst);
     bool invalid = !(m > 0.0f);
     float gbest = -INFINITY;
     int nc = 0;
@@ -160,6 +161,7 @@
     if (to_exact) { o.exact_list[wbase[2 * 16 + wave] + __popcll(mk_e & below)] = (int)n; o.keys[n] = ~0ull; }
     if (to_rescan) { int pos = wbase[0 * 16 + wave] + __popcll(mk_r & below); o.rescan_list[pos] = (int)n; o.rescan_cnt[pos] = 0; o.thr_out[n] = thr; }
     if (to_multi) o.multi_list[wbase[1 * 16 + wave] + __popcll(mk_m & below)] = (int)n;
+    if (settled != nullptr) settled[threadIdx.x] = (!oob && !to_exact && !to_rescan && !to_multi) ? (int)best : -1;
     if (oob) return;
     if (!to_exact && !to_rescan && !to_multi) {
         o.idx[n] = (int64_t)best;
@@ -167,10 +169,10 @@
     }
 }
 
-template <bool AGENT>
+template <bool AGENT, bool ASTATS>
 __device__ __forceinline__ void decide_rows(int64_t n, bool oob, const VqCbStats *st, int Dp, int metric, int nslices,
                                             const float *rec, const float *xh2, const float *rho2, int64_t Np,
-                                            const VqDecideOut &o, int *wcount, int *wbase, const float *rece2) {
+                                            const VqDecideOut &o, int *wcount, int *wbase, const float *rece2, int *settled) {
     if (rece2 != nullptr) {
         switch (nslices) {
 #define VQ_DECIDE_CASE(NSL) case NSL: decide_rows_impl<NSL, AGENT, true>(n, oob, st, Dp, metric, nslices, rec, xh2, rho2, Np, o, wcount, wbase, rece2); break;
@@ -181,10 +183,10 @@
         return;
     }
     switch (nslices) {
-#define VQ_DECIDE_CASE(NSL) case NSL: decide_rows_impl<NSL, AGENT>(n, oob, st, Dp, metric, nslices, rec, xh2, rho2, Np, o, wcount, wbase); break;
+#define VQ_DECIDE_CASE(NSL) case NSL: decide_rows_impl<NSL, AGENT, false, ASTATS>(n, oob, st, Dp, metric, nslices, rec, xh2, rho2, Np, o, wcount, wbase, nullptr, settled); break;
         VQ_DECIDE_CASE(1) VQ_DECIDE_CASE(2) VQ_DECIDE_CASE(4) VQ_DECIDE_CASE(8) VQ_DECIDE_CASE(16)
 #undef VQ_DECIDE_CASE
-        default: decide_rows_impl<0, AGENT>(n, oob, st, Dp, metric, nslices, rec, xh2, rho2, Np, o, wcount, wbase); break;
+        default: decide_rows_impl<0, AGENT, false, ASTATS>(n, oob, st, Dp, metric, nslices, rec, xh2, rho2, Np, o, wcount, wbase, nullptr, settled); break;
     }
 }
 
diff --git a/vector_quantization_amd/csrc/vqhip_update_kernels.h b/vector_quantization_amd/csrc/vqhip_update_kernels.h
--- a/vector_quantization_amd/csrc/vqhip_update_kernels.h
+++ b/vector_quantization_amd/csrc/vqhip_update_kernels.h
@@ -1,8 +1,4 @@
 #pragma once
-__device__ __forceinline__ void nt_store4(float *q, float a, float b, float c, float d) {
-    __builtin_nontemporal_store(a, q); __builtin_nontemporal_store(b, q + 1);
-    __builtin_nontemporal_store(c, q + 2); __builtin_nontemporal_store(d, q + 3);
-}
 
 template <int DT, int NT>
 __global__ __launch_bounds__(1024) void gather_ste_loss_kernel(const void *x, const float *e, const int64_t *idx, int64_t N,
@@ -76,6 +72,50 @@
                     __hip_atomic_store(ticket, 0, __ATOMIC_RELAXED, __HIP_MEMORY_SCOPE_AGENT);
                 }
             }
+        }
+    }
+}
+
+template <int NT>
+__global__ __launch_bounds__(1024) void decode_listed_kernel(const void *x, const float *e, const int64_t *idx, int64_t N,
+                                                            const int *rescan_list, const int *multi_list, const int *exact_list,
+                                                            const int *counters, const int *rescan_cnt, float *z, float *zste,
+                                                            double *sse, float *mse, float beta, int nprop) {
+    __shared__ double red[16];
+    const int lane = threadIdx.x & 63, wave = threadIdx.x >> 6;
+    const int c0 = counters[0], c1 = counters[1], c2 = counters[2];
+    double s = 0.0;
+    for (int i = (int)blockIdx.x * 16 + wave; i < c0 + c1 + c2; i += (int)gridDim.x * 16) {
+        int n;
+        if (i < c0) {
+            const int cnt = rescan_cnt[i];
+            if (cnt > VQ_RESCAN_CAP || cnt <= 0) continue;
+            n = rescan_list[i];
+        } else if (i < c0 + c1) n = multi_list[i - c0];
+        else n = exact_list[i - c0 - c1];
+        const uint2 t = row256_load_bf16<NT>(x, n, lane);
+        const float4 zv = *(const float4 *)(e + idx[n] * 256 + lane * 4);
+        s += (double)row256_decode<NT>(t, zv, z, zste, n, lane);
+    }
+#pragma unroll
+    for (int off = 32; off >= 1; off >>= 1) s += __shfl_xor(s, off, 64);
+    if (lane == 0) red[wave] = s;
+    __syncthreads();
+    if (threadIdx.x == 0) {
+        double t = 0.0;
+#pragma unroll
+        for (int i = 0; i < 16; ++i) t += red[i];
+        int *ticket = (int *)(sse + 1);
+        const double before = atomicAdd(sse, t);
+        asm volatile("" :: "v"(before) : "memory");
+        if (atomicAdd(ticket, 1) == nprop + (int)gridDim.x - 1) {
+            const double total = __hip_atomic_load(sse, __ATOMIC_RELAXED, __HIP_MEMORY_SCOPE_AGENT);
+            const float mean = (float)(total / ((double)N * 256.0));
+            mse[0] = mean; mse[1] = mean;
+            const float weighted = beta * mean;
+            mse[2] = mean + weighted; mse[3] = 0.0f;
+            __hip_atomic_store(sse, 0.0, __ATOMIC_RELAXED, __HIP_MEMORY_SCOPE_AGENT);
+            __hip_atomic_store(ticket, 0, __ATOMIC_RELAXED, __HIP_MEMORY_SCOPE_AGENT);
         }
     }
 }
diff --git a/vector_quantization_amd/quantizers/vector_quantizer.py b/vector_quantization_amd/quantizers/vector_quantizer.py
--- a/vector_quantization_amd/quantizers/vector_quantizer.py
+++ b/vector_quantization_amd/quantizers/vector_quantizer.py
@@ -203,8 +203,11 @@
         if normalize:
             w_out = w_in if cbs[0]._writes_in_place(weight) else torch.empty_like(w_in)
         beta = self._vqgan_beta()
-        out = train_step.vq_forward(x.detach(), w_in, w_out, self._distance.metric_for(weight.shape[1]), beta, normalize=normalize,
-                                    want_hist=self.training and len(cbs) > 0)
+        if not self.training and not normalize:
+            out = train_step.vq_eval_forward(x.detach(), w_in, self._distance.metric_for(weight.shape[1]), beta)
+        else:
+            out = train_step.vq_forward(x.detach(), w_in, w_out, self._distance.metric_for(weight.shape[1]), beta, normalize=normalize,
+                                        want_hist=self.training and len(cbs) > 0)
         if normalize:
             cbs[0]._publish_weight(weight, w_out)
         done = VF._Computed(xn=out['xn'], z_ste=out['z_ste'], mse=out['mse'], idx=out['idx'])
diff --git a/vector_quantization_amd/train_step.py b/vector_quantization_amd/train_step.py
--- a/vector_quantization_amd/train_step.py
+++ b/vector_quantization_amd/train_step.py
@@ -250,6 +250,31 @@
 
 
 @_on_tensor_device
+def vq_eval_forward(x: torch.Tensor, w: torch.Tensor, metric, beta: float, *, need_z: bool = False, need_ste: bool = True,
+                    z_out: Optional[torch.Tensor] = None, z_ste_out: Optional[torch.Tensor] = None):
+    ops._require_cuda(x, w)
+    L = _lib.lib()
+    x, dt = _latents(x)
+    w = _codebook(w)
+    (N, D), K, dev, m = x.shape, w.shape[0], x.device, METRICS[metric]
+    cos = m in (_lib.METRIC_COS, _lib.METRIC_COS_BF16)
+    out = dict(x=x, idx=torch.empty(N, dtype=torch.int64, device=dev), hist=None, xn=None,
+               xq=torch.empty(N, D, dtype=torch.float32, device=dev) if cos else None,
+               z=z_out if z_out is not None else (torch.empty(N, D, dtype=torch.float32, device=dev) if need_z else None),
+               z_ste=z_ste_out if z_ste_out is not None else (torch.empty(N, D, dtype=torch.float32, device=dev) if need_ste else None),
+               mse=torch.empty(4, dtype=torch.float32, device=dev))
+    for buf in (out['z'], out['z_ste']):
+        assert buf is None or (buf.dtype == torch.float32 and buf.shape == (N, D) and buf.is_contiguous() and buf.device == dev)
+    image = _bytes(L.vqhip_codebook_bytes(K, D), dev)
+    ws = _bytes(L.vqhip_workspace_bytes(N, K, D), dev)
+    check(L.vqhip_vq_eval_forward(x.data_ptr(), dt, w.data_ptr(), N, K, D, m, image.data_ptr(), image.numel(), out['idx'].data_ptr(),
+                                  _p(out['xq']), _p(out['z']), _p(out['z_ste']), out['mse'].data_ptr(), float(beta),
+                                  _mse_scratch(dev).data_ptr(), ws.data_ptr(), ws.numel(), _stream()), 'vqhip_vq_eval_forward')
+    out['prepared'] = ops.PreparedCodebook(image, w, K, D, m)
+    return out
+
+
+@_on_tensor_device
 def vqkd_backward(x: torch.Tensor, xn: torch.Tensor, w: torch.Tensor, idx: torch.Tensor, g_zste: Optional[torch.Tensor],
                   g_loss: Optional[torch.Tensor]) -> torch.Tensor:
     ops._require_cuda(x, xn, w, idx)
```

New measurement: 155.8 million tokens/s. -2.9%, worse.
